# DiamondLightSource/fast-feedback-service

Hardware: AMD Instinct MI355X
Metric: detector frames/s (Eiger-16M 4362x4148 uint16) (higher is better)
Workload: dtype u16; 1 GPU; eiger16m: 4148x4362 uint16, 7x7 dispersion window, 32 frames/step/GPU resident in HBM, spots+centroids returned to host; streams=4, parallelism=single GPU, spot_gather=none (single GPU)

## Files before the change

### fast-feedback-service_amd/csrc/ffs_bench.hip

```cpp
#include "ffs_internal.hpp"

extern "C" int ffs_bench_threshold(ffs_stream* s, const void* device_pixels, size_t pitch, size_t fstride,
                                   uint32_t n_frames, uint32_t iters, float* ms_dense, float* ms_rest) {
    if (!s || !device_pixels || iters == 0) return FFS_ERR_INVALID;
    ffs_ctx* c = s->ctx;
    if (s->busy) {
        c->err = "stream busy";
        return FFS_ERR_INVALID;
    }
    int rc = check_layout(s, pitch, fstride, n_frames);
    if (rc != FFS_OK) return rc;
    HIP_TRY(c, hipSetDevice(c->device));
    s->batch_params = c->params;
    const bool ext = c->params.algorithm == FFS_ALGO_DISPERSION_EXTENDED;
    if (ext) {
        rc = ensure_extended_buffers(s);
        if (rc != FFS_OK) return rc;
    }
    s->ext_e_clean = false;
    const StreamGeometry geo = batch_stream_geometry(s, fstride, n_frames);
    ThresholdArgs ta = make_threshold_args(s, device_pixels, pitch, fstride, n_frames, geo, Rerun{});
    if (!ext && !win_default(c->params) && !window_kernel_for(s, ta)) {
        c->err = "ffs_bench_threshold: threshold_path 2 with a window other than 3,3 has no dense kernel to time";
        return FFS_ERR_INVALID;
    }
    const bool e_sparse = ext && ext_sparse_erode(c->tune);
    ta.eplane_clean = e_sparse ? 1 : 0;
    if (!ext) (void)wave_logs_for(s, ta, geo, Rerun{});
    const Layout& L = c->L;
    std::vector<hipEvent_t> ev(4 * (size_t)iters, nullptr);
    auto cleanup = [&]() { for (hipEvent_t e : ev) if (e) (void)hipEventDestroy(e); };
    for (auto& e : ev)
        if (hipEventCreate(&e) != hipSuccess) {
            cleanup();
            c->err = "hipEventCreate failed";
            return FFS_ERR_DEVICE;
        }
    (void)hipGetLastError();
    hipError_t err = hipSuccess;
    for (uint32_t i = 0; i < iters && err == hipSuccess; ++i) {
        err = hipMemsetAsync(s->d_bits, 0, (size_t)s->max_batch * L.plane_frame_stride, s->st);
        if (err == hipSuccess) err = hipMemsetAsync(s->d_tile_counts, 0, tile_counts_bytes(s), s->st);
        if (err == hipSuccess) err = hipMemsetAsync(s->d_occ, 0, (size_t)s->max_batch * occ_frame_words(L) * 4, s->st);
        if (err == hipSuccess && e_sparse) err = hipMemsetAsync(s->d_eplane, 0, (size_t)s->max_batch * L.plane_frame_stride, s->st);
        if (err != hipSuccess) break;
        launch_dense_kernel(s, ta, geo, n_frames, ev[4 * i], ev[4 * i + 1]);
        err = hipEventRecord(ev[4 * i + 2], s->st);
        launch_dense_rest(s, ta, n_frames);
        if (err == hipSuccess) err = hipEventRecord(ev[4 * i + 3], s->st);
        if (err == hipSuccess) err = hipGetLastError();
    }
    if (err == hipSuccess) err = hipMemsetAsync(s->d_overflow, 0, 4, s->st);
    if (err == hipSuccess) err = hipStreamSynchronize(s->st);
    double t_dense = 0, t_rest = 0;
    for (uint32_t i = 0; i < iters && err == hipSuccess; ++i) {
        float a = 0, b = 0;
        err = hipEventElapsedTime(&a, ev[4 * i], ev[4 * i + 1]);
        if (err == hipSuccess) err = hipEventElapsedTime(&b, ev[4 * i + 2], ev[4 * i + 3]);
        t_dense += a;
        t_rest += b;
    }
    cleanup();
    s->bits_dirty = true;
    s->counts_dirty = true;
    s->occ_dirty = true;
    if (err != hipSuccess) {
        c->err = std::string("ffs_bench_threshold: ") + hipGetErrorString(err);
        return FFS_ERR_DEVICE;
    }
    if (ms_dense) *ms_dense = (float)(t_dense / iters);
    if (ms_rest) *ms_rest = (float)(t_rest / iters);
    return FFS_OK;
}

static int bench_pipeline_impl(ffs_stream* const* streams, uint32_t n_streams, const void* device_pixels, size_t pitch, size_t fstride,
                               uint32_t n_frames, uint32_t steps, int64_t first_frame_id, uint64_t* n_boxes, uint64_t* n_strong) {
    uint64_t boxes = 0, strong = 0;
    std::vector<uint32_t> inflight;
    auto reap = [&]() -> int {
        const ffs_frame_result* res = nullptr;
        uint32_t n = 0;
        const int rc = ffs_wait_impl(streams[inflight.front()], &res, &n);
        inflight.erase(inflight.begin());
        if (rc != FFS_OK) return rc;
        for (uint32_t i = 0; i < n; ++i) { boxes += res[i].n_boxes; strong += res[i].num_strong_pixels; }
        return FFS_OK;
    };
    for (uint32_t step = 0; step < steps; ++step) {
        const uint32_t i = step % n_streams;
        if (inflight.size() == n_streams) {
            const int rc = reap();
            if (rc != FFS_OK) return rc;
        }
        const int rc = ffs_submit_device(streams[i], device_pixels, pitch, fstride, n_frames, first_frame_id + (int64_t)step * n_frames);
        if (rc != FFS_OK) return rc;
        inflight.push_back(i);
    }
    while (!inflight.empty()) {
        const int rc = reap();
        if (rc != FFS_OK) return rc;
    }
    if (n_boxes) *n_boxes = boxes;
    if (n_strong) *n_strong = strong;
    return FFS_OK;
// ... 86 lines not shown
```

### fast-feedback-service_amd/csrc/ffs_context.hip

```cpp
#include <sys/mman.h>

#include "ffs_internal.hpp"
#include "kernels_mask.hpp"

static_assert(sizeof(ReflOut) == sizeof(ffs_reflection), "record layout");
static_assert(offsetof(ReflOut, sum_intensity) == offsetof(ffs_reflection, sum_intensity), "record layout");

thread_local std::string g_create_error;

static void ctx_destroy_internal(ffs_ctx* c);
namespace {
struct Registry {
    std::mutex mu;
    std::unordered_set<const void*> live[3];
    std::atomic<bool> exiting{false};
    bool exit_hook_installed = false;
};
Registry& registry() {
    static Registry* r = new Registry();
    return *r;
}
static void on_process_exit() {
    Registry& r = registry();
    std::vector<ffs_ctx*> ctxs;
// ... 186 lines not shown
                {
                    std::unique_lock<std::mutex> lock(mu);
                    cv.wait(lock, [&] { return stop || generation != seen; });
                    if (stop) return;
                    seen = generation;
                    fn = job;
                    n = n_items;
                    if (fn) active.fetch_add(1);
                }
                if (!fn) continue;
                for (;;) {
                    const uint32_t i = next.fetch_add(1);
                    if (i >= n) break;
                    (*fn)(i);
                    done.fetch_add(1, std::memory_order_release);
                }
                active.fetch_sub(1, std::memory_order_release);
            }
        });
}
void AssemblyPool::run(uint32_t n, const std::function<void(uint32_t)>& fn) {
    {
        std::lock_guard<std::mutex> lock(mu);
        job = &fn;
        n_items = n;
        next.store(0);
        done.store(0);
        ++generation;
    }
    cv.notify_all();
    for (;;) {
        const uint32_t i = next.fetch_add(1);
        if (i >= n) break;
        fn(i);
        done.fetch_add(1, std::memory_order_release);
    }
    while (done.load(std::memory_order_acquire) < n) __builtin_ia32_pause();
    {
        std::lock_guard<std::mutex> lock(mu);
        job = nullptr;
    }
    while (active.load(std::memory_order_acquire) != 0) __builtin_ia32_pause();
}
void AssemblyPool::stop_and_join() {
    {
        std::lock_guard<std::mutex> lock(mu);
        stop = true;
    }
    cv.notify_all();
    for (auto& t : threads)
        if (t.joinable()) t.join();
}
AssemblyPool::~AssemblyPool() { stop_and_join(); }

extern "C" void ffs_ctx_destroy(ffs_ctx* c) {
    if (!c || !handle_take(kHandleCtx, c)) return;
    std::vector<ffs_stream*> streams;
    std::vector<ffs_stack3d*> stacks;
    {
        std::lock_guard<std::mutex> lock(c->stream_mu);
        streams.swap(c->live_streams);
        stacks.swap(c->live_stacks);
    }
    for (ffs_stream* s : streams)
        if (handle_take(kHandleStream, s)) stream_destroy_internal(s);
    for (ffs_stack3d* st : stacks)
        if (handle_take(kHandleStack, st)) {
            g_live_stacks.fetch_sub(1);
            stack3d_free(st);
        }
    ctx_destroy_internal(c);
}

static void ctx_destroy_internal(ffs_ctx* c) {
    (void)hipSetDevice(c->device);
    ahead_stop(c, true);
    for (auto* st : c->stack_pool) stack3d_free(st);
    c->stack_pool.clear();
    if (AssemblyPool* pool = c->assembly.exchange(nullptr)) {
        pool->owner.lock();
        pool->owner.unlock();
        delete pool;
    }
    if (c->d_maskbits) (void)hipFree(c->d_maskbits);
    if (c->d_ginfo) (void)hipFree(c->d_ginfo);
    if (c->d_mmap) (void)hipFree(c->d_mmap);
    if (c->dense_st) (void)hipStreamDestroy(c->dense_st);
    if (c->dense_st2) (void)hipStreamDestroy(c->dense_st2);
    if (c->d_handoff) (void)hipFree(c->d_handoff);
    if (c->up_st) (void)hipStreamDestroy(c->up_st);
    for (auto st : c->sparse_st) if (st) (void)hipStreamDestroy(st);
    for (auto e : c->chain_ev) if (e) (void)hipEventDestroy(e);
    for (auto& pb : c->pinned_pool) pinned_free(pb);
    delete c;
}

static int rebuild_mask_tables(ffs_ctx* c) {
    const Layout& L = c->L;
    const uint32_t gpitch = ginfo_pitch(L, c->pixel_bytes);
    HIP_TRY(c, hipMemset(c->d_ginfo, 0, (size_t)(L.H + kInfoExtraRows) * gpitch));
    const int groups = L.pitch_px / (c->pixel_bytes == 2 ? 8 : 4);
    (void)hipGetLastError();
    if (c->pixel_bytes == 2)
        hipLaunchKernelGGL(k_build_maps, dim3((groups + 255) / 256, L.H), dim3(256), 0, 0, c->d_maskbits, L.mpitch, L.W, L.H,
                           L.pitch_px, c->d_mmap, c->d_ginfo, gpitch);
    else
        hipLaunchKernelGGL(k_build_maps4, dim3((groups + 255) / 256, L.H), dim3(256), 0, 0, c->d_maskbits, L.mpitch, L.W, L.H,
                           L.pitch_px, c->d_mmap, c->d_ginfo, gpitch);
    HIP_TRY(c, hipGetLastError());
    HIP_TRY(c, hipDeviceSynchronize());
    return FFS_OK;
}

static int ffs_ctx_set_mask_impl(ffs_ctx* c, const uint8_t* host_mask) {
    if (!c) return FFS_ERR_INVALID;
    const Layout& L = c->L;
    std::vector<uint8_t> bits(L.plane_frame_stride, 0);
    const int full = L.W / 8;
    for (int y = 0; y < L.H; ++y) {
        uint8_t* row = bits.data() + (size_t)y * L.mpitch;
        if (host_mask) {
            const uint8_t* m = host_mask + (size_t)y * L.W;
            for (int g = 0; g < full; ++g) {
                uint64_t v;
                std::memcpy(&v, m + 8 * g, 8);
                const uint64_t nz = (((v & 0x7F7F7F7F7F7F7F7Full) + 0x7F7F7F7F7F7F7F7Full) | v) & 0x8080808080808080ull;
                row[g] = (uint8_t)(((nz >> 7) * 0x0102040810204080ull) >> 56);
            }
            for (int x = full * 8; x < L.W; ++x)
                if (m[x]) row[x >> 3] |= (uint8_t)(1u << (x & 7));
        } else {
            std::memset(row, 0xFF, (size_t)full);
            for (int x = full * 8; x < L.W; ++x) row[x >> 3] |= (uint8_t)(1u << (x & 7));
        }
    }
    HIP_TRY(c, hipSetDevice(c->device));
    HIP_TRY(c, hipMemcpy(c->d_maskbits, bits.data(), bits.size(), hipMemcpyHostToDevice));
    return rebuild_mask_tables(c);
}

static int ffs_ctx_get_mask_impl(ffs_ctx* c, uint8_t* host_mask) {
    if (!c || !host_mask) return FFS_ERR_INVALID;
    const Layout& L = c->L;
    std::vector<uint8_t> bits(L.plane_frame_stride);
    HIP_TRY(c, hipSetDevice(c->device));
    HIP_TRY(c, hipMemcpy(bits.data(), c->d_maskbits, bits.size(), hipMemcpyDeviceToHost));
    for (int y = 0; y < L.H; ++y)
        for (int x = 0; x < L.W; ++x)
            host_mask[(size_t)y * L.W + x] = (bits[(size_t)y * L.mpitch + (x >> 3)] >> (x & 7)) & 1;
    return FFS_OK;
}

extern "C" int ffs_ctx_apply_resolution_mask(ffs_ctx* c, float wavelength, float distance_m,
                                             float bcx, float bcy, float psx, float psy, float dmin,
                                             float dmax) {
    if (!c) return FFS_ERR_INVALID;
    HIP_TRY(c, hipSetDevice(c->device));
    const Layout& L = c->L;
    dim3 block(64, 1), grid((L.mpitch + 63) / 64, L.H);
    hipLaunchKernelGGL(k_resolution_mask, grid, block, 0, 0, c->d_maskbits, L.mpitch, L.W, L.H,
                       wavelength, distance_m, bcx, bcy, psx, psy, dmin, dmax);
    HIP_TRY(c, hipGetLastError());
    HIP_TRY(c, hipDeviceSynchronize());
    return rebuild_mask_tables(c);
}

extern "C" int ffs_ctx_set_params(ffs_ctx* c, const ffs_params* p) {
    if (!c || !p) return FFS_ERR_INVALID;
    if (p->kernel_half_x < 0 || p->kernel_half_x > kWinMaxHalf || p->kernel_half_y < 0 || p->kernel_half_y > kWinMaxHalf) {
        c->err = "ffs_ctx_set_params: kernel_half_x / kernel_half_y must be in 1..7 (0 = 3)";
        return FFS_ERR_INVALID;
    }
    const int win_px = (2 * win_half(p->kernel_half_x) + 1) * (2 * win_half(p->kernel_half_y) + 1);
    if (p->min_count < 2 || p->min_count > win_px || p->nsig_b < 0 || p->nsig_s < 0 || p->threshold < 0) {
        c->err = "ffs_ctx_set_params: need 2 <= min_count <= (2*kernel_half_x+1)*(2*kernel_half_y+1) (49 for the 7x7 window), "
                 "nsig_b >= 0, nsig_s >= 0, threshold >= 0";
        return FFS_ERR_INVALID;
    }
    if (p->algorithm == FFS_ALGO_DISPERSION_EXTENDED && !win_default(*p)) {
        c->err = "ffs_ctx_set_params: the extended dispersion algorithm needs the 7x7 window (kernel_half_x = kernel_half_y = 3): "
                 "its erosion and final pass derive from it";
        return FFS_ERR_INVALID;
    }
    if ((p->algorithm != FFS_ALGO_DISPERSION && p->algorithm != FFS_ALGO_DISPERSION_EXTENDED)
        || (p->extended_flavour != 0 && p->extended_flavour != 1)) {
        c->err = "ffs_ctx_set_params: unknown algorithm / extended_flavour";
        return FFS_ERR_INVALID;
    }
    c->params = *p;
    return FFS_OK;
}

extern "C" int ffs_ctx_device_layout(const ffs_ctx* c, size_t* pitch, size_t* fstride) {
    if (!c) return FFS_ERR_INVALID;
    if (pitch) *pitch = c->L.pitch;
    if (fstride) *fstride = c->L.frame_stride;
    return FFS_OK;
}

extern "C" int ffs_ctx_set_tuning(ffs_ctx* c, const char* key, long long value) {
    if (!c || !key) return FFS_ERR_INVALID;
    Tuning& t = c->tune;
    const std::string k = key;
    auto in = [&](long long lo, long long hi) { return value >= lo && value <= hi; };
    bool ok = true;
    if (k == "threshold_path") { if ((ok = in(0, 2))) t.threshold_path = (int)value; }
    else if (k == "window_kernel") { if ((ok = in(0, 1))) t.window_kernel = (int)value; }
    else if (k == "ext_first_pass") { if ((ok = value == 0 || value == 2)) t.ext_first_pass = (int)value; }
    else if (k == "sparse_stage") { if ((ok = in(1, 3))) t.sparse_stage = (int)value; }
    else if (k == "device_lists") { if ((ok = in(0, 2))) t.device_lists = (int)value; }
    else if (k == "strong_log") { if ((ok = in(0, 1))) t.strong_log = (int)value; }
    else if (k == "chain_runs") { if ((ok = in(0, 2))) t.chain_runs = (int)value; }
    else if (k == "dense_overlap") { if ((ok = in(0, 1))) t.dense_overlap = (int)value; }
    else if (k == "stream_prio") { if ((ok = in(0, 3))) t.stream_prio = (int)value; }
    else if (k == "wait_ahead") { if ((ok = in(0, 1))) t.wait_ahead = (int)value; }
    else if (k == "assembly_threads") { if ((ok = in(1, 31))) t.assembly_threads = (int)value; }
    else if (k == "sparse_bands") { if ((ok = in(0, 2))) t.sparse_bands = (int)value; }
    else if (k == "sparse_priority") {
        if ((ok = in(0, 2) && c->n_streams_made == 0)) {
            int lo = 0, hi = 0;
            HIP_TRY(c, hipSetDevice(c->device));
            HIP_TRY(c, hipDeviceGetStreamPriorityRange(&lo, &hi));
            const int prio = value == 0 ? hi : value == 1 ? lo : (lo + hi) / 2;
            for (auto& sp : c->sparse_st) {
                if (sp) (void)hipStreamDestroy(sp);
                sp = nullptr;
                HIP_TRY(c, hipStreamCreateWithPriority(&sp, hipStreamNonBlocking, prio));
            }
            t.sparse_priority = (int)value;
        }
    }
    else if (k == "sched") { if ((ok = (value == 0 || value == 3) && c->n_streams_made == 0)) t.sched = (int)value; }
    else if (k == "chain_first") { if ((ok = in(0, 64))) t.chain_first = (int)value; }
    else if (k == "bright_cap") { if ((ok = in(0, kBrightCap))) t.bright_cap = (int)value; }
    else if (k == "frames_per_group") { if ((ok = in(1, 1 << 30))) t.frames_per_group = (int)value; }
    else if (k == "target_waves") { if ((ok = in(1, 1 << 24))) t.target_waves = value; }
    else if (k == "stream_bands") { if ((ok = in(0, 4096))) t.stream_bands = (int)value; }
    else if (k == "dense_mask") { if ((ok = in(0, 1))) t.dense_mask = (int)value; }
    else if (k == "occupancy_bitmap") { if ((ok = in(0, 1))) t.occupancy_bitmap = (int)value; }
    else if (k == "direct_records") { if ((ok = in(0, 1) && c->n_streams_made == 0)) t.direct_records = (int)value; }
    else if (k == "decode_in_dense_stream") { if ((ok = in(0, 1))) t.decode_in_dense_stream = (int)value; }
    else if (k == "ext_fused") { if ((ok = in(0, 1))) t.ext_fused = (int)value; }
    else if (k == "ext_erode") { if ((ok = in(0, 2))) t.ext_erode = (int)value; }
    else if (k == "ext_e_sparse") { if ((ok = in(0, 1))) t.ext_e_sparse = (int)value; }
    else if (k == "ext_rest_aside") { if ((ok = in(0, 1))) t.ext_rest_aside = (int)value; }
    else if (k == "band_taper") { if ((ok = in(0, 99))) t.band_taper = (int)value; }
    else if (k == "rows_ahead") { if ((ok = in(2, 4))) t.rows_ahead = (int)value; }
    else if (k == "ccl_grid") { if ((ok = in(1, 1024))) t.ccl_grid = (int)value; }
    else {
        c->err = "ffs_ctx_set_tuning: unknown key '" + k + "'";
        return FFS_ERR_INVALID;
    }
    if (!ok) {
        c->err = "ffs_ctx_set_tuning: value out of range for '" + k + "' (sched / direct_records: before the first stream is created)";
        return FFS_ERR_INVALID;
    }
    return FFS_OK;
}


extern "C" void ffs_stream_destroy(ffs_stream* s) {
    if (!s || !handle_take(kHandleStream, s)) return;
    {
        ffs_ctx* c = s->ctx;
        std::lock_guard<std::mutex> lock(c->stream_mu);
        auto& v = c->live_streams;
        v.erase(std::remove(v.begin(), v.end(), s), v.end());
    }
    stream_destroy_internal(s);
}

void stream_destroy_internal(ffs_stream* s) {
    (void)hipSetDevice(s->ctx->device);
    if (s->job.joinable()) s->job.join();
    (void)ahead_take(s);
    gather_scratch_free(s);
    mark_idle(s);
#ifdef FFS_EXPERIMENTS
    if (s->phase_n) {
        const double k = 1.0 / (double)s->phase_n;
        std::fprintf(stderr, "[ffs exp] sparse launch, %llu frames: init %.1f | L1 / E %.1f | S + L2 %.1f | X U %.1f | P %.1f | R %.1f | whole %.1f us per frame\n",
                     s->phase_n, s->phase_sum[0] * k, s->phase_sum[1] * k, s->phase_sum[2] * k, s->phase_sum[3] * k, s->phase_sum[4] * k, s->phase_sum[5] * k, s->phase_sum[6] * k);
    }
    if (s->h_phase_ts) (void)hipHostFree(s->h_phase_ts);
#endif
    if (s->big) stream_destroy_internal(s->big);
    if (s->st_up && s->st_up != s->st) (void)hipStreamSynchronize(s->st_up);
    if (s->st) (void)hipStreamSynchronize(s->st);
    if (s->st_shared && s->ctx->dense_st2) (void)hipStreamSynchronize(s->ctx->dense_st2);
    if (s->st2 && s->st2 != s->st) { (void)hipStreamSynchronize(s->st2); if (!s->st2_shared) (void)hipStreamDestroy(s->st2); }
    if (s->h_pack_tab) (void)hipHostFree(s->h_pack_tab);
    void* dev[] = {s->d_slab, s->d_pack_k, s->d_pack_i, s->d_pack_tab, s->d_comp, s->d_tab, s->d_ext_pair[0], s->d_ext_pair[1], s->d_wlog, s->d_wlog_n, s->d_wpix,
                   s->d_band_hdr, s->d_band_acc, s->d_band_seam, s->d_bo_frames, s->d_bo_lane, s->d_bo_map, s->d_bo_state};
    for (void* p : dev)
        if (p) (void)hipFree(p);
    void* host[] = {s->h_tab, s->h_bo_frames, s->h_counts, s->h_recs, s->h_list_k, s->h_list_i, s->h_mask};
    for (void* p : host)
        if (p) (void)hipHostFree(p);
    if (s->h_img) {
        std::lock_guard<std::mutex> lock(s->ctx->stream_mu);
        s->ctx->pinned_pool.push_back(s->h_img_buf);
    }
    for (auto& e : s->ev)
        if (e) (void)hipEventDestroy(e);
    if (s->ev_pack) (void)hipEventDestroy(s->ev_pack);
    if (s->ev_sent) (void)hipEventDestroy(s->ev_sent);
    if (s->st && !s->st_shared) (void)hipStreamDestroy(s->st);
    delete s;
}

extern "C" int ffs_stream_create(ffs_ctx* c, ffs_stream** out) {
    if (!c || !out) return FFS_ERR_INVALID;
    const int rc = stream_create_sized(c, c->max_batch, c->cap, c->max_comp, out);
    if (rc != FFS_OK) return rc;
    {
        std::lock_guard<std::mutex> lock(c->stream_mu);
        c->live_streams.push_back(*out);
    }
    handle_add(kHandleStream, *out);
    return FFS_OK;
}

int stream_create_sized(ffs_ctx* c, uint32_t max_batch, uint32_t cap, uint32_t max_comp, ffs_stream** out) {
    *out = nullptr;
    HIP_TRY(c, hipSetDevice(c->device));
    ffs_stream* s = new (std::nothrow) ffs_stream();
    if (!s) return FFS_ERR_NOMEM;
    s->ctx = c;
    s->max_batch = max_batch;
// ... 192 lines not shown
```

### fast-feedback-service_amd/csrc/ffs_device.h

```cpp
#pragma once
#include <hip/hip_runtime.h>
#include <stdint.h>

#include "launch_geometry.hpp"

#ifdef FFS_EXPERIMENTS
#define FFS_DBG(args, bit) (((args).dbg & (bit)) != 0)
#define FFS_STOP_AFTER(A, phase) if ((A).stop_after == (phase)) return
#define FFS_PHASE_TS(A, idx) do { if ((A).phase_ts && threadIdx.x == 0) (A).phase_ts[(size_t)blockIdx.x * 8 + (idx)] = wall_clock64(); } while (0)
#else
#define FFS_PHASE_TS(A, idx) do {} while (0)
#define FFS_DBG(args, bit) false
#define FFS_STOP_AFTER(A, phase) do {} while (0)
#endif

namespace ffsamd {

constexpr int kInfoExtraRows = 3;

constexpr int kWlogCap = 256;
constexpr int kTileRows = 8;
constexpr int kExactListCap = 2048;

struct ThresholdArgs {
    const void* image;
    uint64_t frame_stride;
    uint32_t pitch;
    const uint8_t* maskbits;
    uint8_t* bits;
    uint8_t* strong_bytes;
    uint32_t* tile_counts;
    int W, H, pitch_px;
    uint32_t mpitch, bpitch;
    uint64_t plane_frame_stride, bytes_frame_stride;
    int n_strips, band_rows, n_bands, n_tiles;
    int band_rows2, band_split;
    float kS;
    float kB;
    int min_count;
    double nsig_b, nsig_s, threshold;
    double nsig_b2, nsig_s2;
    long long max_valid;
    int int_pred;
    uint32_t ib2, is2;
    uint32_t thr_floor;
    int bright_to_plane;
    uint8_t* dplane;
    uint8_t* eplane;
    int eplane_clean;
    int ext_strips, ext_band_rows, ext_bands;
    int ext_flavour;
    int ext_variant;
    const uint8_t* ginfo;
    const uint8_t* mmap;
    uint32_t gpitch;
    int gpf;
    int n_frames;
    int group_frames;
    int s_strips, s_band_rows, s_bands;
    uint32_t* bright_n;
    uint2* bright_list;
    uint32_t bright_cap;
    uint32_t* overflow;
    uint32_t* occ;
    uint32_t occ_frame_words;
    uint32_t occ_spr;
    int dense_mask;
    uint2* wlog;
    uint32_t* wlog_n;
    uint4* wpix;
    uint32_t* handoff;
    uint32_t handoff_seq;
    int dbg_prio;
    int dbg;
    int kx, ky;
    int w_strips, w_band_rows, w_bands;
    float w_kS, w_kB;
};

__host__ __device__ inline uint32_t stream_units(const ThresholdArgs& a) { return stream_units_of(a.n_bands, a.n_strips); }
__host__ __device__ inline uint32_t stream_chunk(const ThresholdArgs& a) { return stream_chunk_of(a.n_bands, a.n_strips); }
__device__ __forceinline__ bool stream_unit(const ThresholdArgs& a, uint32_t bid, int& strip, int& band) {
    return stream_unit_of(bid, a.n_bands, a.n_strips, strip, band);
}
__host__ __device__ inline uint32_t log_slot(const ThresholdArgs& a, uint32_t y, uint32_t band, uint32_t strip) {
    return log_slot_of(a.n_bands, a.n_strips, y, band, strip);
}

constexpr uint32_t kOvfStrongCap = 1u;
constexpr uint32_t kOvfCompCap = 2u;
constexpr uint32_t kOvfCorruptLz4 = 4u;
constexpr uint32_t kOvfBrightList = 8u;
constexpr uint32_t kOvfRuns = 16u;
constexpr uint32_t kOvfWaveLog = 32u;
constexpr uint32_t kOvfLdsForest = 64u;
constexpr uint32_t kOvfBandPlan = 128u;
constexpr uint32_t kOvfCorruptByteOffset = 256u;
constexpr uint32_t kRecTooSmall = 1u;
constexpr uint32_t kRecTooSpread = 2u;

constexpr int kSummaryWords = 8;
constexpr uint32_t kSumBoxes = 0, kSumStrongFiltered = 1, kSumReflections = 2, kSumFilteredSize = 3, kSumFilteredSep = 4;
__host__ __device__ constexpr size_t counts_strong_at(size_t) { return 0; }
__host__ __device__ constexpr size_t counts_comp_at(size_t B) { return B; }
__host__ __device__ constexpr size_t counts_summary_at(size_t B) { return 2 * B; }
__host__ __device__ constexpr size_t counts_status_at(size_t B) { return (2 + kSummaryWords) * B; }
__host__ __device__ constexpr size_t counts_frame_flags_at(size_t B) { return counts_status_at(B) + 1; }
__host__ __device__ constexpr size_t counts_device_words(size_t B) { return counts_status_at(B) + 1; }
__host__ __device__ constexpr size_t counts_host_words(size_t B) { return counts_frame_flags_at(B) + B; }

struct CompAcc2 {
    unsigned long long sum_i, sum_xi, sum_yi, peak;
    uint32_t x_min, x_max, y_min, y_max;
    uint32_t num_pixels, pad;
};

struct WireRec2 {
    uint16_t x_min, x_max, y_min, y_max;
    uint32_t npx_flags;
    float com_x, com_y;
    uint16_t peak_x, peak_y;
    uint32_t peak_intensity;
    float peak_centroid_distance;
    unsigned long long sum_intensity;
};

struct CclArgs {
    const void* image;
    uint64_t frame_stride;
    uint32_t pitch;
    uint8_t* bits;
    int clear_bits;
    const uint32_t* tile_counts;
    uint32_t* num_strong;
    uint32_t* row_off;
    uint32_t* list_k;
    uint32_t* list_i;
    uint32_t* parent;
    uint32_t* comp_id;
    uint32_t* n_comp;
    uint32_t* overflow;
    int W, H, pitch_px;
    uint32_t mpitch;
    uint64_t plane_frame_stride;
    int n_tiles;
    uint32_t cap;
    uint32_t max_comp;
    int pixel_bytes;
    CompAcc2* acc2;
    uint32_t* summary;
    uint8_t* strong_bytes;
    uint32_t bpitch;
    uint64_t bytes_frame_stride;
    int dense_bytes;
    int need_lists;
    uint32_t* occ;
    uint32_t occ_frame_words, occ_spr;
    int use_occ;
};

struct CompAcc {
    unsigned long long sum_i;
    unsigned long long sum_xi;
    unsigned long long sum_yi;
    unsigned long long sum_zi;
    unsigned long long peak;
// ... 58 lines not shown
```

### fast-feedback-service_amd/csrc/ffs_internal.hpp

```cpp
#pragma once
#include <algorithm>
#include <atomic>
#include <chrono>
#include <condition_variable>
#include <functional>
#include <cmath>
#include <cstdio>
#include <cstdlib>
#include <cstring>
#include <deque>
#include <map>
#include <mutex>
#include <new>
#include <string>
#include <thread>
#include <unordered_set>
#include <vector>

#include <hip/hip_runtime.h>
#include <hip/hip_ext.h>

#include "ffs_hip.h"
#include "ffs_device.h"
#include "tuning.hpp"
// ... 3 lines not shown
extern thread_local std::string g_create_error;

struct ThreadError {
    static std::string& text() {
        static thread_local std::string t;
        return t;
    }
    const ThreadError& operator=(const std::string& m) const { text() = m; return *this; }
    const ThreadError& operator=(const char* m) const { text() = m; return *this; }
    const char* c_str() const { return text().c_str(); }
    operator std::string() const { return text(); }
};


struct ffs_stack3d;

struct AssemblyPool {
    std::vector<std::thread> threads;
    std::mutex mu;
    std::condition_variable cv;
    std::mutex owner;
    const std::function<void(uint32_t)>* job = nullptr;
    uint32_t n_items = 0;
    std::atomic<uint32_t> next{0}, done{0};
    std::atomic<int> active{0};
    uint64_t generation = 0;
    bool stop = false;
    void start(int n_threads);
    void run(uint32_t n, const std::function<void(uint32_t)>& fn);
    void stop_and_join();
    ~AssemblyPool();
};

struct PinnedBuf {
    uint8_t* p = nullptr;
    size_t bytes = 0;
    void* map_base = nullptr;
    size_t map_len = 0;
};
PinnedBuf pinned_alloc(size_t bytes);
void pinned_free(PinnedBuf& b);

struct AheadThread {
    std::thread th;
    std::mutex mu;
    std::condition_variable cv_work, cv_done;
    std::deque<ffs_stream*> q;
    bool stop = false;
};

struct ffs_ctx {
    int device = 0;
    Tuning tune;
    Layout L{};
    int pixel_bytes = 2;
    uint32_t max_batch = 1;
    uint32_t cap = 0;
    uint32_t max_comp = 0;
    int n_tiles = 0;
    ffs_params params{};
    uint8_t* d_maskbits = nullptr;
    uint8_t* d_ginfo = nullptr;
    uint8_t* d_mmap = nullptr;
    hipStream_t dense_st = nullptr;
    hipStream_t dense_st2 = nullptr;
    uint32_t* d_handoff = nullptr;
    std::mutex dense_mu;
    uint32_t handoff_seq = 0;
    int handoff_last = -1;
    hipStream_t up_st = nullptr;
    hipStream_t sparse_st[2] = {nullptr, nullptr};
    int n_streams_made = 0;
    std::mutex stream_mu;
    std::vector<ffs_stream*> live_streams;
    std::vector<ffs_stack3d*> live_stacks;
    std::vector<ffs_stack3d*> stack_pool;
    std::vector<struct PinnedBuf> pinned_pool;
    std::atomic<int> inflight{0};
    static constexpr int kChainEvents = 16;
    hipEvent_t chain_ev[kChainEvents] = {};
    std::atomic<uint32_t> chain_ev_next{0};
    std::atomic<int> chain_ev_newest{-1};
    bool chain_ok = false;
    std::atomic<AssemblyPool*> assembly{nullptr};
    std::atomic<AheadThread*> ahead{nullptr};
    ThreadError err;
};

struct OverflowFrame;

constexpr uint32_t kBrightCap = 1u << 20;

struct ffs_stream {
    ffs_ctx* ctx = nullptr;
    uint32_t max_batch = 1;
    uint32_t cap = 0;
    uint32_t max_comp = 0;
    ffs_stream* big = nullptr;
    std::vector<OverflowFrame> ovf;
    bool lists_valid = true;
    bool log_off = false;
    uint2* d_wlog = nullptr;
    uint32_t* d_wlog_n = nullptr;
    uint4* d_wpix = nullptr;
    size_t wlog_waves = 0;
    uint4* d_band_hdr = nullptr;
    uint8_t* d_band_acc = nullptr;
    uint32_t* d_band_seam = nullptr;
    uint32_t band_slots = 0;
    uint32_t band_backoff = 0;
    uint32_t path_bits = 0;
    uint32_t reruns = 0;
    bool runs_overflowed = false;
    uint32_t *d_pack_k = nullptr, *d_pack_i = nullptr;
    StackSlice *d_pack_tab = nullptr, *h_pack_tab = nullptr;
    hipEvent_t ev_pack = nullptr;
    hipEvent_t ev_sent = nullptr;
    int ev_sent_dev = -1;
    bool sent_pending = false;
    hipStream_t st = nullptr;
    hipStream_t st_up = nullptr;
    bool st2_shared = false;
    bool st_shared = false;
    hipStream_t st2 = nullptr;
    hipEvent_t ev[7] = {};
    uint8_t* d_slab = nullptr;
    uint8_t* d_img = nullptr;
    uint8_t* d_bits = nullptr;
    uint8_t* d_sbytes = nullptr;
    uint8_t *d_dplane = nullptr, *d_eplane = nullptr;
    uint8_t* d_dplane2 = nullptr;
    uint8_t* d_eplane2 = nullptr;
    uint8_t* d_ext_pair[2] = {nullptr, nullptr};
    bool dplane2_clean = false;
    bool eplane2_clean = false;
    bool ext_e_clean = false;
    uint8_t* d_comp = nullptr;
    uint2 *d_tab = nullptr, *h_tab = nullptr;
    uint32_t dec_blocks = 0, dec_last = 0, dec_tail = 0, dec_block_elems = 0;
    uint4 *d_bo_frames = nullptr, *h_bo_frames = nullptr;
    uint2 *d_bo_lane = nullptr, *d_bo_map = nullptr;
    uint4* d_bo_state = nullptr;
    size_t bo_tiles_cap = 0;
    uint32_t spec_recs_per_frame = 256;
    uint64_t spec_recs_copied = 0;
    std::thread job;
    int job_rc = 0;
    std::string job_err;
    uint32_t *d_tile_counts = nullptr, *d_num_strong = nullptr, *d_row_off = nullptr;
    uint2* d_bright = nullptr;
    uint32_t *d_list_k = nullptr, *d_list_i = nullptr, *d_parent = nullptr;
    uint32_t *d_n_comp = nullptr, *d_overflow = nullptr, *d_summary = nullptr;
    CompAcc2* d_acc2 = nullptr;
    uint32_t* d_chunk_roots = nullptr;
    ReflOut* d_recs = nullptr;
    uint8_t* h_img = nullptr;
    size_t h_img_bytes = 0;
    PinnedBuf h_img_buf;
    size_t d_comp_bytes = 0;
    uint32_t* h_counts = nullptr;
    ReflOut* h_recs = nullptr;
    uint32_t* d_occ = nullptr;
    uint32_t* h_counts_dev = nullptr;
    bool ev1_pending = false;
    bool ev3_is_ev4 = false;
    bool dev_input = false;
// ... 31 lines not shown
    std::vector<float> centres_n;
    int ahead_state = 0;
};

struct OverflowFrame {
    uint32_t frame = 0;
    ffs_frame_result res{};
    std::vector<ffs_box> boxes;
    std::vector<ffs_reflection> refls;
    std::vector<uint32_t> k, inten;
};

static inline const OverflowFrame* overflow_frame(const std::vector<OverflowFrame>* ovf, uint32_t f) {
    if (ovf)
        for (const OverflowFrame& o : *ovf)
            if (o.frame == f) return &o;
    return nullptr;
}

template <typename F>
static int guarded(ffs_ctx* c, F&& body) {
    try {
        return body();
    } catch (const std::exception& e) {
        if (c) c->err = std::string("exception inside libffs_hip: ") + e.what();
        else g_create_error = std::string("exception inside libffs_hip: ") + e.what();
        return FFS_ERR_NOMEM;
    } catch (...) {
        if (c) c->err = "unknown exception inside libffs_hip";
        return FFS_ERR_NOMEM;
    }
}

#define HIP_TRY(ctx, expr)                                                              \
    do {                                                                                \
        hipError_t e_ = (expr);                                                         \
        if (e_ != hipSuccess) {                                                         \
            (ctx)->err = std::string(#expr) + ": " + hipGetErrorString(e_);             \
            return e_ == hipErrorOutOfMemory ? FFS_ERR_NOMEM : FFS_ERR_DEVICE;          \
        }                                                                               \
    } while (0)

struct Rerun {
    int threshold_path = -1;
    bool plane = false;
    bool no_bands = false;
    bool grid = false;
};
static inline bool ext_sparse_erode(const Tuning& t) { return t.ext_erode != 0 && t.ext_e_sparse; }
constexpr int kWinMaxHalf = 7;
static inline int win_half(int v) { return v ? v : 3; }
static inline bool win_default(const ffs_params& p) { return win_half(p.kernel_half_x) == 3 && win_half(p.kernel_half_y) == 3; }
static inline uint32_t occ_frame_words(const Layout& L) { return (uint32_t)(((uint64_t)L.H * (L.mpitch / 16) + 31) / 32 + 2); }
static inline size_t tile_counts_bytes(const ffs_stream* s) { return (((size_t)s->max_batch * s->ctx->n_tiles + 2) * 4 + 255) / 256 * 256; }
static inline void mark_busy(ffs_stream* s) {
    if (!s->busy) ++s->ctx->inflight;
    s->busy = true;
}
static inline void mark_idle(ffs_stream* s) {
    if (s->busy) --s->ctx->inflight;
    s->busy = false;
}
template <typename T>
static hipError_t dmalloc(T** p, size_t n_bytes) {
    return hipMalloc(reinterpret_cast<void**>(p), n_bytes + 256);
}

enum HandleKind { kHandleCtx = 0, kHandleStream = 1, kHandleStack = 2 };
void handle_add(HandleKind kind, const void* h);
bool handle_take(HandleKind kind, const void* h);
bool handle_live(HandleKind kind, const void* h);
bool process_exiting();
static inline bool stream_handle_ok(const ffs_stream* s) {
    if (handle_live(kHandleStream, s)) return true;
    g_create_error = "stale ffs_stream handle: the stream was destroyed (with its context, or by ffs_stream_destroy)";
    return false;
}
void stream_destroy_internal(ffs_stream* s);

int stream_create_sized(ffs_ctx* c, uint32_t max_batch, uint32_t cap, uint32_t max_comp, ffs_stream** out);
int ensure_host_staging(ffs_stream* s, size_t bytes);
size_t default_staging_bytes(const ffs_stream* s);
bool chain_prepare_device();
StreamGeometry batch_stream_geometry(const ffs_stream* s, size_t fstride, uint32_t n_frames);
ThresholdArgs make_threshold_args(ffs_stream* s, const void* img, size_t pitch, size_t fstride, uint32_t n_frames, const StreamGeometry& g, const Rerun& how);
int check_layout(ffs_stream* s, size_t pitch, size_t fstride, uint32_t n_frames);
int ensure_extended_buffers(ffs_stream* s);
int enqueue_batch(ffs_stream* s, const void* d_img, size_t pitch, size_t fstride, uint32_t n, const ffs_params* snapshot = nullptr,
                  const Rerun& how = Rerun{});
extern std::atomic<int> g_live_stacks;
bool wave_logs_for(ffs_stream* s, ThresholdArgs& a, const StreamGeometry& g, const Rerun& how);
void launch_dense_kernel(ffs_stream* s, const ThresholdArgs& a, const StreamGeometry& g, uint32_t n_frames, hipEvent_t start, hipEvent_t stop,
                         bool plane_clean = false, bool counts_clean = false);
void launch_dense_rest(ffs_stream* s, const ThresholdArgs& a, uint32_t n_frames);
bool window_kernel_for(const ffs_stream* s, const ThresholdArgs& a);
int ffs_wait_impl(ffs_stream* s, const ffs_frame_result** results, uint32_t* n_results);
void ahead_register(ffs_stream* s);
int ahead_take(ffs_stream* s);
void ahead_stop(ffs_ctx* c, bool destroy);
void stack3d_free(ffs_stack3d* st);
void gather_scratch_free(ffs_stream* s);
```

### fast-feedback-service_amd/csrc/ffs_submit.hip

```cpp
#include "ffs_internal.hpp"
#include "kernels_threshold.hpp"
#include "kernels_extended.hpp"
#include "kernels_stream.hpp"
#include "kernels_ccl.hpp"
#include "kernels_chain.hpp"
#include "kernels_band.hpp"
#include "kernels_decode.hpp"
#include "kernels_byteoffset.hpp"
#include "kernels_window.hpp"

bool chain_prepare_device() {
    const hipError_t e1 = hipFuncSetAttribute(reinterpret_cast<const void*>(&k_frame_chain<uint16_t>), hipFuncAttributeMaxDynamicSharedMemorySize, kChainDynBytes);
    const hipError_t e2 = hipFuncSetAttribute(reinterpret_cast<const void*>(&k_frame_chain<uint32_t>), hipFuncAttributeMaxDynamicSharedMemorySize, kChainDynBytes);
    const hipError_t e3 = hipFuncSetAttribute(reinterpret_cast<const void*>(&k_frame_chain<uint16_t, true>), hipFuncAttributeMaxDynamicSharedMemorySize, kChainDynBytes);
    const hipError_t e4 = hipFuncSetAttribute(reinterpret_cast<const void*>(&k_frame_chain<uint16_t, false, true>), hipFuncAttributeMaxDynamicSharedMemorySize, kChainDynBytes);
    const hipError_t e5 = hipFuncSetAttribute(reinterpret_cast<const void*>(&k_frame_chain<uint32_t, false, true>), hipFuncAttributeMaxDynamicSharedMemorySize, kChainDynBytes);
    (void)hipGetLastError();
    return e1 == hipSuccess && e2 == hipSuccess && e3 == hipSuccess && e4 == hipSuccess && e5 == hipSuccess;
}

static void set_buffers(ThresholdArgs& a, const ffs_stream* s, const void* img, size_t pitch, size_t fstride, const Rerun& how) {
    const ffs_ctx* c = s->ctx;
    const Layout& L = c->L;
    const ffs_params& p = s->batch_params;
    a.image = img;
    a.frame_stride = fstride;
    a.pitch = (uint32_t)pitch;
    a.maskbits = c->d_maskbits;
    a.bits = s->d_bits;
    a.strong_bytes = s->d_sbytes;
    a.tile_counts = s->d_tile_counts;
    a.W = L.W;
    a.H = L.H;
    a.pitch_px = L.pitch_px;
    a.mpitch = L.mpitch;
    a.bpitch = L.bpitch;
    a.plane_frame_stride = L.plane_frame_stride;
    a.bytes_frame_stride = L.bytes_frame_stride;
    a.n_tiles = c->n_tiles;
    a.bright_to_plane = how.threshold_path >= 0 ? how.threshold_path : c->tune.threshold_path;
    a.overflow = s->d_overflow;
    a.bright_n = s->d_tile_counts + tile_counts_bytes(s) / 4 - 1;
    a.bright_list = s->d_bright;
    a.bright_cap = std::min<uint32_t>(kBrightCap, (uint32_t)c->tune.bright_cap);
    a.occ = s->d_occ;
    a.occ_frame_words = occ_frame_words(L);
    a.occ_spr = L.mpitch / 16;
    a.dense_mask = (p.want_strong_mask || c->tune.dense_mask || a.bright_to_plane) ? 1 : 0;
#ifdef FFS_EXPERIMENTS
    a.dbg = c->tune.exp.k1_debug;
    if (a.dbg & 16) a.dense_mask = 1;
    if (a.dbg & 8) a.dense_mask = 0;
#endif
    a.dbg_prio = c->tune.stream_prio;
    a.ginfo = c->d_ginfo;
    a.mmap = c->d_mmap;
    a.gpitch = ginfo_pitch(L, c->pixel_bytes);
    a.gpf = groups_per_row(L, c->pixel_bytes);
    a.dplane = s->d_dplane;
    a.eplane = s->d_eplane;
    a.eplane_clean = s->ext_e_clean ? 1 : 0;
    a.ext_variant = (c->pixel_bytes == 2 && how.threshold_path < 0) ? c->tune.ext_first_pass : 0;
}
static void set_predicate(ThresholdArgs& a, const ffs_params& p) {
    a.kS = (float)(p.nsig_s * p.nsig_s * (1.0 - 1.0 / 65536.0));
    a.kB = (float)(p.nsig_b * (1.0 - 1.0 / 1048576.0));
    a.min_count = p.min_count;
    a.nsig_b = p.nsig_b;
    a.nsig_s = p.nsig_s;
    a.nsig_b2 = p.nsig_b * p.nsig_b;
    a.nsig_s2 = p.nsig_s * p.nsig_s;
    a.threshold = p.threshold;
    a.max_valid = p.max_valid;
    {
        const double b2 = p.nsig_b * p.nsig_b, s2 = p.nsig_s * p.nsig_s;
        a.int_pred = (b2 == std::floor(b2) && s2 == std::floor(s2) && b2 <= 1024.0 && s2 <= 1024.0 && p.threshold < 2147483648.0
                      && std::sqrt(b2) == p.nsig_b && std::sqrt(s2) == p.nsig_s) ? 1 : 0;
        a.ib2 = a.int_pred ? (uint32_t)b2 : 0u;
        a.is2 = a.int_pred ? (uint32_t)s2 : 0u;
        a.thr_floor = a.int_pred ? (uint32_t)std::floor(p.threshold) : 0u;
    }
    a.kx = win_half(p.kernel_half_x);
    a.ky = win_half(p.kernel_half_y);
    a.w_kS = (std::isfinite(p.nsig_s) && p.nsig_s <= 1024.0) ? (float)(p.nsig_s * p.nsig_s * (1.0 - 1.0 / 65536.0)) : 0.0f;
    a.w_kB = (std::isfinite(p.nsig_b) && p.nsig_b <= 1024.0) ? (float)(p.nsig_b * p.nsig_b * (1.0 - 1.0 / 65536.0)) : 0.0f;
    a.ext_flavour = p.extended_flavour;
}
static void set_geometry(ThresholdArgs& a, uint32_t n_frames, const StreamGeometry& g, const WindowGeometry& w, const ExtGeometry& e) {
    a.n_frames = (int)n_frames;
    a.group_frames = g.group_frames;
    a.n_strips = g.n_strips;
    a.n_bands = g.n_bands;
    a.band_rows = g.band_rows;
    a.band_rows2 = g.band_rows2;
    a.band_split = g.band_split;
    a.w_strips = w.w_strips;
    a.w_band_rows = w.w_band_rows;
    a.w_bands = w.w_bands;
    a.ext_strips = e.ext_strips;
    a.ext_band_rows = e.ext_band_rows;
    a.ext_bands = e.ext_bands;
}
StreamGeometry batch_stream_geometry(const ffs_stream* s, size_t fstride, uint32_t n_frames) {
    return stream_geometry(s->ctx->L, s->ctx->pixel_bytes, fstride, n_frames, s->ctx->tune);
}
ThresholdArgs make_threshold_args(ffs_stream* s, const void* img, size_t pitch, size_t fstride, uint32_t n_frames, const StreamGeometry& g, const Rerun& how) {
    ThresholdArgs a{};
    set_buffers(a, s, img, pitch, fstride, how);
    set_predicate(a, s->batch_params);
    set_geometry(a, n_frames, g, window_geometry(s->ctx->L, n_frames, a.ky), ext_geometry(s->ctx->L, n_frames));
    return a;
}

static dim3 stream_grid(const ThresholdArgs& a, const StreamGeometry& g) {
    return dim3(8u * stream_chunk(a), (unsigned)g.n_groups);
}

using StreamKernel = void (*)(ThresholdArgs);
static StreamKernel stream_kernel(const ffs_ctx* c, bool dense_mask, bool extended) {
    const int rows = std::clamp(c->tune.rows_ahead, 2, c->pixel_bytes == 4 ? 3 : 4);
    if (c->pixel_bytes == 4) return dense_mask ? k_stream_u32<2, true> : rows == 3 ? k_stream_u32<3, false> : k_stream_u32<2, false>;
    if (extended) return dense_mask ? k_stream_u16<2, true, true> : k_stream_u16<2, true, false>;
    if (dense_mask) return k_stream_u16<2, false, true>;
    return rows == 4 ? k_stream_u16<4, false, false> : rows == 3 ? k_stream_u16<3, false, false> : k_stream_u16<2, false, false>;
}
static void launch_stream(ffs_stream* s, const ThresholdArgs& a, const StreamGeometry& g, hipEvent_t start, hipEvent_t stop, hipStream_t st = nullptr) {
    hipExtLaunchKernelGGL(stream_kernel(s->ctx, a.dense_mask != 0, false), stream_grid(a, g), dim3(64), 0, st ? st : s->st, start, stop, 0, a);
}
bool window_kernel_for(const ffs_stream* s, const ThresholdArgs& a) {
    return s->batch_params.algorithm == FFS_ALGO_DISPERSION && a.bright_to_plane != 2
           && (!win_default(s->batch_params) || s->ctx->tune.window_kernel == 1);
}
template <typename PixelT>
static void launch_window_t(const ThresholdArgs& a, dim3 grid, hipStream_t st, hipEvent_t start, hipEvent_t stop) {
    const size_t lds = win_ring_bytes((int)sizeof(PixelT), a.ky);
    switch (a.kx) {
        case 1: hipExtLaunchKernelGGL((k_window<PixelT, 1>), grid, dim3(64), lds, st, start, stop, 0, a); break;
        case 2: hipExtLaunchKernelGGL((k_window<PixelT, 2>), grid, dim3(64), lds, st, start, stop, 0, a); break;
        case 3: hipExtLaunchKernelGGL((k_window<PixelT, 3>), grid, dim3(64), lds, st, start, stop, 0, a); break;
        case 4: hipExtLaunchKernelGGL((k_window<PixelT, 4>), grid, dim3(64), lds, st, start, stop, 0, a); break;
        case 5: hipExtLaunchKernelGGL((k_window<PixelT, 5>), grid, dim3(64), lds, st, start, stop, 0, a); break;
        case 6: hipExtLaunchKernelGGL((k_window<PixelT, 6>), grid, dim3(64), lds, st, start, stop, 0, a); break;
        default: hipExtLaunchKernelGGL((k_window<PixelT, 7>), grid, dim3(64), lds, st, start, stop, 0, a); break;
    }
}
static void launch_window(ffs_stream* s, const ThresholdArgs& a, uint32_t n_frames, hipEvent_t start, hipEvent_t stop, hipStream_t st = nullptr) {
    const dim3 grid((unsigned)(a.w_strips * a.w_bands), n_frames);
    if (!st) st = s->st;
    if (s->ctx->pixel_bytes == 4) launch_window_t<uint32_t>(a, grid, st, start, stop);
    else launch_window_t<uint16_t>(a, grid, st, start, stop);
}
static void launch_bright_fix(ffs_stream* s, const ThresholdArgs& a, hipStream_t st) {
    if (s->ctx->pixel_bytes == 4) hipLaunchKernelGGL(k_bright_fix<uint32_t>, dim3(32), dim3(256), 0, st, a);
    else hipLaunchKernelGGL(k_bright_fix<uint16_t>, dim3(32), dim3(256), 0, st, a);
}
static void launch_exact(ffs_stream* s, const ThresholdArgs& a, uint32_t n_frames, hipStream_t st) {
    const dim3 grid((unsigned)a.n_tiles, n_frames);
    if (a.kx != 3 || a.ky != 3) {
        if (s->ctx->pixel_bytes == 4) hipLaunchKernelGGL(k_exact_w<uint32_t>, grid, dim3(256), 0, st, a);
        else hipLaunchKernelGGL(k_exact_w<uint16_t>, grid, dim3(256), 0, st, a);
        return;
    }
    if (s->ctx->pixel_bytes == 4) hipLaunchKernelGGL(k_exact<uint32_t>, grid, dim3(256), 0, st, a);
    else hipLaunchKernelGGL(k_exact<uint16_t>, grid, dim3(256), 0, st, a);
}

static bool ext_stream_first(const ThresholdArgs& a) { return a.ext_variant >= 2; }

static void launch_ext_first(ffs_stream* s, const ThresholdArgs& a, const StreamGeometry& g, uint32_t n_frames, hipEvent_t start, hipEvent_t stop, bool fix_here = true,
                             bool plane_clean = false, bool counts_clean = false) {
    if (ext_stream_first(a)) {
        if (!plane_clean) (void)hipMemsetAsync(a.dplane, 0, (size_t)n_frames * a.plane_frame_stride, s->st);
        if (!counts_clean) (void)hipMemsetAsync(a.tile_counts, 0, tile_counts_bytes(s), s->st);
        hipExtLaunchKernelGGL(stream_kernel(s->ctx, a.dense_mask != 0, true), stream_grid(a, g), dim3(64), 0, s->st, start, stop, 0, a);
        if (fix_here) hipLaunchKernelGGL((k_bright_fix<uint16_t, true>), dim3(32), dim3(256), 0, s->st, a);
        return;
    }
    dim3 g1((unsigned)(a.ext_strips * a.ext_bands), n_frames);
    if (s->ctx->pixel_bytes == 2) hipExtLaunchKernelGGL(k_ext_first<uint16_t>, g1, dim3(64), 0, s->st, start, stop, 0, a);
    else hipExtLaunchKernelGGL(k_ext_first<uint32_t>, g1, dim3(64), 0, s->st, start, stop, 0, a);
}
static void launch_ext_rest(ffs_stream* s, const ThresholdArgs& a, uint32_t n_frames, hipStream_t st) {
    const bool u16 = s->ctx->pixel_bytes == 2;
    if (!ext_stream_first(a)) (void)hipMemsetAsync(a.strong_bytes, 0, (size_t)n_frames * a.bytes_frame_stride, st);
    dim3 g3((unsigned)a.n_tiles, n_frames);
    if (u16 && s->ctx->tune.ext_fused) {
        hipLaunchKernelGGL(k_ext_erode_final, g3, dim3(256), (size_t)(kTileRows + 10) * a.mpitch, st, a);
        return;
    }
    const int erode = s->ctx->tune.ext_erode;
    if (erode != 0) {
        const unsigned strips = (a.mpitch / 4 + 61) / 62, rows = erode == 1 ? 32 : 16;
        const dim3 ge(strips * 8u * (((unsigned)((a.H + rows - 1) / rows) + 7u) / 8u), n_frames);
// ... 54 lines not shown
    return true;
}
bool wave_logs_for(ffs_stream* s, ThresholdArgs& a, const StreamGeometry& g, const Rerun& how) {
    if (!wave_logs_possible(s, a, how)) return false;
    size_t slots = stream_log_slots(g);
    if (slots > s->wlog_waves) slots = std::max(slots, max_stream_log_slots(s->ctx->L, s->ctx->pixel_bytes, a.frame_stride, s->max_batch, s->ctx->tune));
    if (!ensure_wave_logs(s, slots)) return false;
    a.wlog = s->d_wlog;
    a.wlog_n = s->d_wlog_n;
    a.wpix = s->d_wpix;
    return true;
}

void launch_dense_kernel(ffs_stream* s, const ThresholdArgs& a, const StreamGeometry& g, uint32_t n_frames, hipEvent_t start, hipEvent_t stop, bool plane_clean, bool counts_clean) {
    if (s->batch_params.algorithm == FFS_ALGO_DISPERSION_EXTENDED) launch_ext_first(s, a, g, n_frames, start, stop, true, plane_clean, counts_clean);
    else if (window_kernel_for(s, a)) launch_window(s, a, n_frames, start, stop);
    else launch_stream(s, a, g, start, stop);
}
void launch_dense_rest(ffs_stream* s, const ThresholdArgs& a, uint32_t n_frames) {
    if (s->batch_params.algorithm == FFS_ALGO_DISPERSION_EXTENDED) launch_ext_rest(s, a, n_frames, s->st);
    else if (window_kernel_for(s, a)) return;
    else if (a.bright_to_plane) launch_exact(s, a, n_frames, s->st);
    else if (!a.wlog) launch_bright_fix(s, a, s->st);
}

int check_layout(ffs_stream* s, size_t pitch, size_t fstride, uint32_t n_frames) {
    ffs_ctx* c = s->ctx;
    if (n_frames == 0 || n_frames > s->max_batch) {
        c->err = "n_frames must be in 1..max_batch";
        return FFS_ERR_INVALID;
    }
    if (pitch % 16 || pitch < (size_t)c->L.pitch_px * c->pixel_bytes || pitch >= (1ull << 32)
        || fstride < pitch * c->L.H || (pitch * c->L.H) >= (1ull << 32)) {
        c->err = "device layout: pitch must be a multiple of 16 bytes and >= round_up(width,128)*pixel_bytes; "
                 "frame_stride >= pitch*height";
        return FFS_ERR_INVALID;
    }
    return FFS_OK;
}

#ifdef FFS_EXPERIMENTS
__global__ void k_dummy_spin(uint32_t ticks, uint32_t* sink) {
    extern __shared__ uint32_t s_dummy[];
    const uint64_t t0 = wall_clock64();
    uint32_t it = 0;
    while (wall_clock64() - t0 < ticks && it < (1u << 20)) { __builtin_amdgcn_s_sleep(20); ++it; }
    if (it == 0xFFFFFFFFu) { s_dummy[threadIdx.x] = it; *sink = s_dummy[0]; }
}
#endif

static bool ensure_band_buffers(ffs_stream* s, uint32_t slots) {
    if (slots <= s->band_slots) return true;
    if (s->d_band_hdr) {
        (void)hipFree(s->d_band_hdr); (void)hipFree(s->d_band_acc); (void)hipFree(s->d_band_seam);
        s->d_band_hdr = nullptr; s->d_band_acc = nullptr; s->d_band_seam = nullptr;
    }
    s->band_slots = 0;
    if (hipMalloc(reinterpret_cast<void**>(&s->d_band_hdr), (size_t)slots * sizeof(uint4)) != hipSuccess
        || hipMalloc(reinterpret_cast<void**>(&s->d_band_acc), (size_t)slots * kBandCompStride * sizeof(ChainAcc)) != hipSuccess
        || hipMalloc(reinterpret_cast<void**>(&s->d_band_seam), (size_t)slots * 2 * kBandSeamCap * 4) != hipSuccess) {
        (void)hipGetLastError();
        return false;
    }
    s->band_slots = slots;
    return true;
}
static bool band_stage_for(ffs_stream* s, const StreamGeometry& g, size_t fstride, uint32_t n_frames) {
    const ffs_ctx* c = s->ctx;
    if (!band_plan_holds(g, c->L, c->pixel_bytes)) return false;
    uint32_t slots = band_slots(g, n_frames);
    if (slots > s->band_slots) slots = std::max(slots, max_band_slots(c->L, c->pixel_bytes, fstride, s->max_batch, c->tune));
    return ensure_band_buffers(s, slots);
}


#define FFS_TRY(expr)                    \
    do {                                 \
        const int rc_ = (expr);          \
        if (rc_ != FFS_OK) return rc_;   \
    } while (0)

struct BatchPlan {
    uint32_t n = 0;
    bool wait_upload = false;
    bool counts_were_clean = false;
    bool ext = false;
    bool ext_sparse_erode = false;
    bool window = false;
    bool list_path = false;
    bool aside = false;
    bool will_chain = false;
    bool runs_ok = false;
    bool dense_batch = false;
    bool use_log = false;
    bool runs_launch = false;
    bool need_lists = false;
    bool banded = false;
    bool chain_first = false;
    bool want_dense_bytes = false;
    StreamGeometry geo{};
    ThresholdArgs ta{};
    ThresholdArgs ta_launch{};
    BandSplit band;
    uint32_t path_bits = 0;
};

static BatchPlan plan_batch(ffs_stream* s, const void* d_img, size_t pitch, size_t fstride, uint32_t n, const Rerun& how) {
    ffs_ctx* c = s->ctx;
    const Layout& L = c->L;
    const ffs_params& p = s->batch_params;
    BatchPlan P;
    P.n = n;
    P.wait_upload = s->st_up != s->st && !s->dev_input;
    P.counts_were_clean = !s->counts_dirty;
    P.ext = p.algorithm == FFS_ALGO_DISPERSION_EXTENDED;
    P.ext_sparse_erode = ext_sparse_erode(c->tune);
    P.geo = batch_stream_geometry(s, fstride, n);
    P.ta = make_threshold_args(s, d_img, pitch, fstride, n, P.geo, how);
    P.window = !P.ext && window_kernel_for(s, P.ta);
    P.list_path = !P.ext && !P.ta.bright_to_plane && !P.window;
    P.want_dense_bytes = P.window ? (p.want_strong_mask || c->tune.dense_mask)
                                  : (P.list_path || (P.ext && ext_stream_first(P.ta))) ? P.ta.dense_mask != 0 : true;
    const bool can_chain = c->tune.sparse_stage >= 2 && L.H <= 65535 && c->chain_ok && s->direct_recs && s->h_counts_dev
                           && c->n_tiles <= kChainMaxTiles && L.H <= kChainMaxRows;
    P.runs_ok = c->pixel_bytes == 2 && L.W <= kChainRunMaxW && c->tune.chain_runs != 0 && !s->runs_overflowed;
    if (can_chain && c->tune.sparse_stage == 2 && s->n_frames > 0) {
        uint32_t prev_max = 0;
        for (uint32_t f = 0; f < s->n_frames; ++f) prev_max = std::max(prev_max, s->h_counts[counts_strong_at(s->max_batch) + f]);
        P.dense_batch = prev_max > (uint32_t)kChainLdsEntries;
    }
    P.will_chain = can_chain && (!P.dense_batch || P.runs_ok) && !how.grid;
    P.ta_launch = P.ta;
    P.use_log = P.list_path && P.will_chain && !P.dense_batch && wave_logs_for(s, P.ta_launch, P.geo, how);
#ifdef FFS_EXPERIMENTS
    if (c->tune.exp.chain_skip) P.will_chain = false;
#endif
    P.runs_launch = P.will_chain && !P.use_log && P.runs_ok && (P.dense_batch || c->tune.chain_runs == 2);
    P.aside = !P.ext && s->st2 != s->st;
    const int depth = c->inflight.load() + (s->busy ? 0 : 1);
    P.need_lists = p.want_strong_list || c->tune.device_lists == 1 || (c->tune.device_lists == 2 && g_live_stacks.load() > 0);
    const bool depth_ok = c->tune.sparse_bands >= 2 || depth >= 4 || depth <= 1 || c->n_streams_made >= 4;
    P.banded = P.use_log && c->tune.sparse_bands != 0 && depth_ok && !P.need_lists && !P.ta.dense_mask && !how.no_bands && s->band_backoff == 0
               && band_stage_for(s, P.geo, fstride, n);
    if (P.banded) P.band = band_split(P.geo);
    P.chain_first = P.list_path && P.aside && P.will_chain && !P.banded && c->tune.chain_first > 0 && depth <= c->tune.chain_first;
    P.path_bits = (P.use_log ? FFS_PATH_WAVE_LOGS : 0u) | (P.will_chain && !P.banded ? FFS_PATH_FRAME_CHAIN : 0u) | (P.banded ? FFS_PATH_BANDS : 0u)
                  | (P.runs_launch ? FFS_PATH_RUNS : 0u) | (!P.will_chain ? FFS_PATH_GRID_KERNELS : 0u) | (P.ext ? FFS_PATH_EXTENDED : 0u)
                  | (P.window ? FFS_PATH_WINDOW : 0u);
    return P;
}

static int take_extended_planes(ffs_stream* s, bool& plane_clean) {
    plane_clean = false;
    s->ext_e_clean = false;
    if (s->batch_params.algorithm != FFS_ALGO_DISPERSION_EXTENDED) return FFS_OK;
    FFS_TRY(ensure_extended_buffers(s));
    std::swap(s->d_dplane, s->d_dplane2);
    std::swap(s->d_eplane, s->d_eplane2);
    plane_clean = s->dplane2_clean;
    s->ext_e_clean = s->dplane2_clean && s->eplane2_clean && ext_sparse_erode(s->ctx->tune);
    s->dplane2_clean = false;
    s->eplane2_clean = false;
    return FFS_OK;
}

static int reset_for_batch(ffs_stream* s, const BatchPlan& plan, bool& dense_resets) {
    ffs_ctx* c = s->ctx;
    const Layout& L = c->L;
    dense_resets = false;
    if (plan.wait_upload && plan.ext) HIP_TRY(c, hipStreamWaitEvent(s->st, s->ev[1], 0));
    if (!plan.ext && s->bits_dirty) {
        HIP_TRY(c, hipMemsetAsync(s->d_bits, 0, (size_t)s->max_batch * L.plane_frame_stride, s->st));
        dense_resets = true;
    }
    if (!plan.ext && s->counts_dirty) {
        HIP_TRY(c, hipMemsetAsync(s->d_tile_counts, 0, tile_counts_bytes(s), s->st));
        dense_resets = true;
    }
    if (s->occ_dirty) {
        HIP_TRY(c, hipMemsetAsync(s->d_occ, 0, (size_t)s->max_batch * occ_frame_words(L) * 4, s->st));
        s->occ_dirty = false;
        dense_resets = true;
    }
    s->counts_dirty = true;
    s->bits_dirty = true;
    return FFS_OK;
}

static int wait_for_upload(ffs_stream* s, const BatchPlan& plan, hipStream_t st) {
    if (plan.wait_upload) HIP_TRY(s->ctx, hipStreamWaitEvent(st, s->ev[1], 0));
    return FFS_OK;
}
static int sparse_stream_follows(ffs_stream* s, bool ev2_on_dispatch) {
    if (!ev2_on_dispatch) HIP_TRY(s->ctx, hipEventRecord(s->ev[2], s->st));
    if (s->st2 != s->st) HIP_TRY(s->ctx, hipStreamWaitEvent(s->st2, s->ev[2], 0));
    return FFS_OK;
}

static int launch_stream_overlapped(ffs_stream* s, const BatchPlan& plan, hipEvent_t ev_start, bool& launched) {
    ffs_ctx* c = s->ctx;
    launched = false;
// ... 198 lines not shown
            BA.sub = plan.band.sub;
            BA.sub_rows = plan.band.sub_rows;
            const dim3 gb((unsigned)(plan.ta_launch.n_bands * BA.sub), n);
            if (c->pixel_bytes == 2) hipExtLaunchKernelGGL(k_band_cc<uint16_t>, gb, dim3(64), 0, s->st2, c->chain_ev[slot], nullptr, 0, BA);
            else hipExtLaunchKernelGGL(k_band_cc<uint32_t>, gb, dim3(64), 0, s->st2, c->chain_ev[slot], nullptr, 0, BA);
            hipLaunchKernelGGL(k_frame_merge, dim3(n), dim3(kMergeThreads), 0, s->st2, BA);
        } else {
            hipExtLaunchKernelGGL(frame_chain_kernel(plan, c->pixel_bytes), dim3(n), dim3(kChainThreads), kChainDynBytes, s->st2, c->chain_ev[slot], nullptr, 0, A);
        }
        if (plan.aside) c->chain_ev_newest.store(slot);
    }
    HIP_TRY(c, hipGetLastError());
    if (plan.ext && ext_stream_first(plan.ta) && s->st2 != s->st) {
        HIP_TRY(c, hipMemsetAsync(s->d_dplane2, 0, (size_t)s->max_batch * c->L.plane_frame_stride * (plan.ext_sparse_erode ? 2u : 1u), s->st2));
        s->dplane2_clean = true;
        s->eplane2_clean = plan.ext_sparse_erode;
    }
    HIP_TRY(c, hipEventRecord(s->ev[4], s->st2));
    s->ev3_is_ev4 = true;
    s->spec_recs_copied = (uint64_t)s->max_batch * s->max_comp;
    return finish_enqueue(s, n, plan.ext, false);
}

static int launch_grid_stage(ffs_stream* s, const BatchPlan& plan, const CclArgs& ca, SegArgs sa) {
    ffs_ctx* c = s->ctx;
    const uint32_t n = plan.n;
    bool skip_sparse = false;
#ifdef FFS_EXPERIMENTS
    if (c->tune.exp.chain_skip) {
        skip_sparse = true;
        if (c->tune.exp.dummy_us > 0)
            hipLaunchKernelGGL(k_dummy_spin, dim3(c->tune.exp.dummy_wg), dim3(c->tune.exp.dummy_threads),
                               (size_t)c->tune.exp.dummy_lds, s->st2, (uint32_t)c->tune.exp.dummy_us * 100u, s->d_tile_counts);
    }
#endif
    if (!skip_sparse) {
        sa.recs = s->direct_recs ? (void*)s->h_recs_dev : (void*)s->d_recs;
        sa.chunk_roots = s->d_chunk_roots;
        sa.chunks_max = s->cap / kRootChunk + 1;
        const dim3 gseg((unsigned)c->tune.ccl_grid, n), b256(256);
        if (c->pixel_bytes == 2) hipLaunchKernelGGL(k_emit_list_w<uint16_t>, dim3(c->n_tiles, n), dim3(64), 0, s->st2, ca);
        else hipLaunchKernelGGL(k_emit_list_w<uint32_t>, dim3(c->n_tiles, n), dim3(64), 0, s->st2, ca);
        hipLaunchKernelGGL(k_union<false>, gseg, b256, 0, s->st2, sa);
        hipLaunchKernelGGL(k_reduce_roots, gseg, b256, 0, s->st2, sa);
        hipLaunchKernelGGL(k_finalize_roots, gseg, b256, 0, s->st2, sa);
    }
    HIP_TRY(c, hipGetLastError());
    HIP_TRY(c, hipEventRecord(s->ev[3], s->st2));
    s->ev3_is_ev4 = false;

    const size_t B = s->max_batch;
    HIP_TRY(c, hipMemcpyAsync(s->h_counts, s->d_num_strong, counts_device_words(B) * 4, hipMemcpyDeviceToHost, s->st2));
    if (s->direct_recs) {
        s->spec_recs_copied = (uint64_t)B * s->max_comp;
    } else {
        s->spec_recs_copied = std::min<uint64_t>((uint64_t)s->spec_recs_per_frame * n, (uint64_t)B * s->max_comp);
        HIP_TRY(c, hipMemcpyAsync(s->h_recs, s->d_recs, s->spec_recs_copied * sizeof(WireRec2), hipMemcpyDeviceToHost, s->st2));
    }
    HIP_TRY(c, hipEventRecord(s->ev[4], s->st2));
    return finish_enqueue(s, n, plan.ext || skip_sparse, skip_sparse);
}

static int launch_sparse_stage(ffs_stream* s, const BatchPlan& plan) {
    const CclArgs ca = make_ccl_args(s, plan);
    const SegArgs sa = make_seg_args(s, plan);
    s->bits_cleared = ca.clear_bits != 0;
    s->lists_valid = !(plan.use_log || plan.runs_launch) || plan.need_lists;
    s->dense_valid = plan.want_dense_bytes;
    s->occ_dirty = !(ca.use_occ && plan.will_chain);
    s->chain_mode = plan.will_chain;
    s->path_bits = plan.path_bits;
    return plan.will_chain ? launch_one_launch_stage(s, plan, ca, sa) : launch_grid_stage(s, plan, ca, sa);
}

int enqueue_batch(ffs_stream* s, const void* d_img, size_t pitch, size_t fstride, uint32_t n, const ffs_params* snapshot, const Rerun& how) {
    s->batch_params = snapshot ? *snapshot : s->ctx->params;
    s->cur_img = d_img;
    s->cur_pitch = pitch;
    s->cur_fstride = fstride;
    (void)hipGetLastError();
    bool ext_plane_clean = false;
    FFS_TRY(take_extended_planes(s, ext_plane_clean));
    const BatchPlan plan = plan_batch(s, d_img, pitch, fstride, n, how);
    if (plan.use_log && s->band_backoff > 0 && !how.no_bands) --s->band_backoff;
    bool dense_resets = false;
    FFS_TRY(reset_for_batch(s, plan, dense_resets));
    FFS_TRY(launch_threshold_stage(s, plan, dense_resets, ext_plane_clean));
    return launch_sparse_stage(s, plan);
}

extern "C" int ffs_submit_device(ffs_stream* s, const void* device_pixels, size_t pitch, size_t fstride,
                                 uint32_t n_frames, int64_t first_frame_id) {
    if (!s || !device_pixels || !stream_handle_ok(s)) return FFS_ERR_INVALID;
    ffs_ctx* c = s->ctx;
    if (s->busy) {
        c->err = "stream already has a batch in flight: call ffs_wait() first";
        return FFS_ERR_INVALID;
    }
    int rc = check_layout(s, pitch, fstride, n_frames);
    if (rc != FFS_OK) return rc;
    HIP_TRY(c, hipSetDevice(c->device));
    s->dev_input = true;
    s->ev1_pending = true;
    s->first_id = first_frame_id;
    s->reruns = 0;
    rc = enqueue_batch(s, device_pixels, pitch, fstride, n_frames);
    if (rc == FFS_OK) ahead_register(s);
    return rc;
}

extern "C" int ffs_submit(ffs_stream* s, const void* host_pixels, uint32_t n_frames, int64_t first_frame_id) {
    if (!s || !host_pixels || !stream_handle_ok(s)) return FFS_ERR_INVALID;
    ffs_ctx* c = s->ctx;
    if (s->busy) {
        c->err = "stream already has a batch in flight: call ffs_wait() first";
        return FFS_ERR_INVALID;
    }
    if (n_frames == 0 || n_frames > s->max_batch) {
        c->err = "n_frames must be in 1..max_batch";
        return FFS_ERR_INVALID;
    }
    const Layout& L = c->L;
    HIP_TRY(c, hipSetDevice(c->device));
    s->dev_input = false;
    HIP_TRY(c, hipEventRecord(s->ev[0], s->st_up));
    const size_t row = (size_t)L.W * c->pixel_bytes;
    HIP_TRY(c, hipMemcpy2DAsync(s->d_img, L.pitch, host_pixels, row, row, (size_t)L.H * n_frames,
                                hipMemcpyHostToDevice, s->st_up));
    HIP_TRY(c, hipEventRecord(s->ev[1], s->st_up));
    s->first_id = first_frame_id;
    s->reruns = 0;
    const int rc = enqueue_batch(s, s->d_img, L.pitch, L.frame_stride, n_frames);
    if (rc == FFS_OK) ahead_register(s);
    return rc;
}



static int ensure_decode_buffers(ffs_stream* s) {
    ffs_ctx* c = s->ctx;
    if (s->d_tab) return FFS_OK;
    const size_t es = c->pixel_bytes, nelem = (size_t)c->L.W * c->L.H;
    const size_t block = (size_t)kDecBlockBytes / es;
    const size_t n_full = nelem / block, rem = nelem - n_full * block;
    s->dec_block_elems = (uint32_t)block;
    s->dec_blocks = (uint32_t)(n_full + (rem >= 8 ? 1 : 0));
    s->dec_last = (uint32_t)(rem >= 8 ? rem / 8 * 8 : block);
    s->dec_tail = (uint32_t)(rem % 8);
    const size_t tab_bytes = (size_t)s->max_batch * (s->dec_blocks + 1) * sizeof(uint2);
    if (dmalloc(&s->d_tab, tab_bytes) != hipSuccess
        || hipHostMalloc(reinterpret_cast<void**>(&s->h_tab), tab_bytes, hipHostMallocDefault) != hipSuccess) {
        (void)hipGetLastError();
        c->err = "allocation of the compressed-chunk buffers failed";
        return FFS_ERR_NOMEM;
    }
    return FFS_OK;
}

static inline uint32_t be32(const uint8_t* p) {
    return ((uint32_t)p[0] << 24) | ((uint32_t)p[1] << 16) | ((uint32_t)p[2] << 8) | p[3];
}

static int stage_chunks(ffs_stream* s, int codec, const void* const* chunks, const size_t* chunk_bytes, uint32_t n,
                        std::vector<size_t>& base) {
    ffs_ctx* c = s->ctx;
    const Layout& L = c->L;
// ... 370 lines not shown
```

### fast-feedback-service_amd/csrc/kernels_band.hpp

```cpp
#pragma once
#include "kernels_chain.hpp"

namespace ffsamd {

constexpr int kBandChunks = 8;
constexpr int kBandEntries = 64 * kBandChunks;
constexpr int kBandPx = 768;
constexpr int kBandPer = kBandPx / 64;
constexpr int kBandSlots = 64;
constexpr int kBandCompStride = 256;
constexpr int kBandSeamCap = 256;
constexpr int kBandItems = (kBandPx - kBandEntries) / 2;
constexpr int kMergeThreads = 256;
constexpr int kMergeCap = 4096;
constexpr int kMergeSeamLds = 8;
constexpr int kMergeLabels = 2;
constexpr int kMergePer = kMergeCap / kMergeThreads;
static_assert(sizeof(ChainAcc) == 56 && kBandSlots * (int)sizeof(ChainAcc) <= kBandCw * 4, "the accumulators take the counters' LDS");
static_assert(kBandEntries + 2 * kBandItems <= kBandPx && kBandMaxRows % 2 == 0, "LDS plan");

struct BandArgs {
    ChainArgs A;
    int sub, sub_rows;
    uint4* hdr;
    ChainAcc* acc;
    uint32_t* seam;
};

template <typename PixelT>
__global__ __launch_bounds__(64) void k_band_cc(const BandArgs B) {
    const ThresholdArgs& T = B.A.t;
    const CclArgs& a = B.A.c;
    if (T.dbg_prio & 2) __builtin_amdgcn_s_setprio(3);
    __shared__ uint32_t s_lst[16];
    __shared__ uint32_t s_row[kBandMaxRows + 2];
    __shared__ __align__(16) uint32_t s_cw[kBandCw];
    __shared__ __align__(8) uint2 s_ent[kBandEntries];
    __shared__ uint16_t s_x[kBandPx];
    __shared__ uint8_t s_y[kBandPx];
    __shared__ PixelT s_i[kBandPx];
    __shared__ uint32_t s_par[kBandPx];
    __shared__ uint32_t s_flag;

    const int band = (int)blockIdx.x / B.sub, sub = (int)blockIdx.x - band * B.sub, frame = blockIdx.y, lane = threadIdx.x;
    const uint32_t W = (uint32_t)a.W;
    constexpr uint32_t kGroupPx = sizeof(PixelT) == 2 ? 8u : 4u;
    const uint32_t l_y = (uint32_t)frame / (uint32_t)T.group_frames;
    const uint32_t l_fe = (uint32_t)frame - l_y * (uint32_t)T.group_frames;
    const uint32_t gsep = (uint32_t)T.gpf + 1u, G0 = l_fe * gsep, G1 = G0 + (uint32_t)T.gpf - 1u;
    const uint32_t l_s0 = G0 / (uint32_t)kSOwned;
    const uint32_t l_ns = min(G1 / (uint32_t)kSOwned - l_s0 + 1u, 16u);
    const uint32_t wave0 = log_slot(T, l_y, (uint32_t)band, l_s0);
    const int sb1 = min(band_first_row(band + 1, T.band_rows, T.band_rows2, T.band_split), a.H);
    const int yb0 = min(band_first_row(band, T.band_rows, T.band_rows2, T.band_split) + sub * B.sub_rows, sb1);
    const int yb1 = min(yb0 + B.sub_rows, sb1);
    const uint32_t rows = (uint32_t)(yb1 - yb0);
    const uint8_t* img = (const uint8_t*)a.image + (uint64_t)frame * a.frame_stride;
    const size_t slot = (size_t)frame * (size_t)gridDim.x + (size_t)blockIdx.x;

    FFS_STOP_AFTER(B.A, 10);
    if (lane == 0) s_flag = (rows > (uint32_t)kBandMaxRows || rows * l_ns > (uint32_t)kBandCw) ? kOvfBandPlan : 0u;
    for (uint32_t i = lane; i < min(rows * l_ns, (uint32_t)kBandCw); i += 64) s_cw[i] = 0;
    for (uint32_t i = lane; i < kBandEntries; i += 64) s_par[i] = 0;
    __syncthreads();

    uint32_t cnt = 0;
    if ((uint32_t)lane < l_ns && rows != 0) {
        cnt = T.wlog_n[wave0 + (uint32_t)lane];
        if (cnt > (uint32_t)kWlogCap) { atomicOr(&s_flag, kOvfWaveLog); cnt = (uint32_t)kWlogCap; }
    }
    const uint32_t incl0 = wave_inclusive_scan(cnt);
    if (lane < 16) s_lst[lane] = incl0 - cnt;
    const uint32_t nb = (uint32_t)__builtin_amdgcn_readlane((int)incl0, 63);
    if (nb > (uint32_t)kBandEntries) atomicOr(&s_flag, kOvfBandPlan);
    __syncthreads();
    uint32_t n = 0, ncomp = 0, n_top = 0, n_bot = 0;
    if (s_flag == 0 && nb != 0) {
        {
            uint2 ent[kBandChunks];
#pragma unroll
            for (int c = 0; c < kBandChunks; ++c) {
                const uint32_t f = (uint32_t)(c * 64 + lane);
                ent[c] = make_uint2(0xFFFFFFFFu, 0xFFFF0000u);
                if (f < nb) {
                    uint32_t k = 0;
                    for (uint32_t j = 1; j < l_ns; ++j) k += f >= s_lst[j] ? 1u : 0u;
                    ent[c] = T.wlog[(uint64_t)(wave0 + k) * kWlogCap + (f - s_lst[k])];
                    ent[c].y = ((ent[c].y >> 16) != l_fe || (int)(ent[c].x >> 16) < yb0 || (int)(ent[c].x >> 16) >= yb1) ? 0xFFFF0000u : (k << 16) | (ent[c].y & 0xFFFFu);
                }
            }
#pragma unroll
            for (int c = 0; c < kBandChunks; ++c)
                if ((uint32_t)(c * 64) < nb) s_ent[c * 64 + lane] = ent[c];
        }
        __syncthreads();
        FFS_STOP_AFTER(B.A, 12);
        const uint32_t nchunks = (nb + 63u) / 64u;
        auto mine_of = [](uint2 v) -> bool { return (v.y >> 16) != 0xFFFFu; };
        auto load_px = [&](uint32_t c) -> uint4 {
            uint4 px = make_uint4(0u, 0u, 0u, 0u);
            if (c < nchunks) {
                const uint32_t f = c * 64u + (uint32_t)lane;
                const uint2 v = s_ent[f];
                if (f < nb && mine_of(v) && (v.y & 0xFFFFu)) px = T.wpix[(uint64_t)(wave0 + (v.y >> 16)) * kWlogCap + (f - s_lst[v.y >> 16])];
            }
            return px;
        };
        const uint4 px0 = load_px(0), px1 = load_px(1);

        {
            uint32_t* items = s_par + kBandEntries;
            uint32_t nm = 0;
            for (uint32_t c = 0; c < nchunks; ++c) {
                const uint2 v = s_ent[c * 64 + lane];
                uint32_t maybe = mine_of(v) ? (v.y >> 8) & 0xFFu & ~v.y : 0u;
                const uint32_t pc = (uint32_t)__popc(maybe);
                const uint32_t inc = wave_inclusive_scan(pc);
                uint32_t q = nm + inc - pc;
                nm += (uint32_t)__builtin_amdgcn_readlane((int)inc, 63);
                while (maybe) {
                    const int b = __ffs((int)maybe) - 1;
                    maybe &= maybe - 1;
                    if (q < (uint32_t)kBandItems) {
                        items[2 * q] = v.x;
                        items[2 * q + 1] = ((c * 64u + (uint32_t)lane) << 3) | (uint32_t)b;
                    }
                    ++q;
                }
            }
            if (nm > (uint32_t)kBandItems) atomicOr(&s_flag, kOvfBandPlan);
            if (nm != 0) {
                __syncthreads();
                for (uint32_t i = lane; i < min(nm, (uint32_t)kBandItems); i += 64) {
                    const uint32_t rg = items[2 * i], sb = items[2 * i + 1];
                    const uint32_t row = rg >> 16, ge = rg & 0xFFFFu, b = sb & 7u;
                    if (exact_strong_lite<PixelT>(T, img, (int)(ge * kGroupPx + b), (int)row)) atomicOr(&s_par[sb >> 3], 1u << b);
                }
// ... 184 lines not shown
                        uint32_t* dst = reinterpret_cast<uint32_t*>(out + c0);
                        const uint32_t* src = reinterpret_cast<const uint32_t*>(s_acc);
                        for (uint32_t w = lane; w < ndw; w += 64) dst[w] = src[w];
                    }
                    __syncthreads();
                }
                n_top = s_row[1] - s_row[0];
                n_bot = s_row[rows] - s_row[rows - 1];
                if (n_top > (uint32_t)kBandSeamCap || n_bot > (uint32_t)kBandSeamCap) atomicOr(&s_flag, kOvfBandPlan);
                uint32_t* seam = B.seam + slot * 2 * kBandSeamCap;
                for (uint32_t j = lane; j < min(n_top, (uint32_t)kBandSeamCap); j += 64) seam[j] = (uint32_t)s_x[j] | ((uint32_t)s_id[j] << 16);
                const uint32_t bb = s_row[rows - 1];
                for (uint32_t j = lane; j < min(n_bot, (uint32_t)kBandSeamCap); j += 64) seam[kBandSeamCap + j] = (uint32_t)s_x[bb + j] | ((uint32_t)s_id[bb + j] << 16);
            }
        }
    }
    __syncthreads();
    if (lane == 0) B.hdr[slot] = make_uint4(n, ncomp, n_top | (n_bot << 16), s_flag | (rows << 16));
}
template __global__ void k_band_cc<uint16_t>(const BandArgs);
template __global__ void k_band_cc<uint32_t>(const BandArgs);

__global__ __launch_bounds__(kMergeThreads) void k_frame_merge(const BandArgs B) {
    const ChainArgs& A = B.A;
    const CclArgs& a = A.c;
    const SegArgs& sa = A.s;
    const ThresholdArgs& T = A.t;
    if (T.dbg_prio & 2) __builtin_amdgcn_s_setprio(3);
    __shared__ uint32_t s_off[kMergeMaxBands + 1];
    __shared__ uint32_t s_par[kMergeCap];
    __shared__ uint16_t s_l2id[kMergeCap];
    __shared__ uint32_t s_touched[kMergeCap / 32];
    __shared__ uint32_t s_wave[kMergeThreads / 64];
    __shared__ uint32_t s_sm[kSummaryWords];
    __shared__ uint32_t s_tot[2];
    __shared__ __align__(16) uint32_t s_out[kMergeLabels * kMergeThreads * (sizeof(WireRec2) / 4)];
    __shared__ __align__(16) uint32_t s_seam[kMergeMaxBands * 2 * kMergeSeamLds];
    const int frame = blockIdx.x, tid = threadIdx.x;
    const uint32_t W = (uint32_t)a.W;
    const uint32_t nbands = (uint32_t)(T.n_bands * B.sub);
    const uint4* hdr = B.hdr + (size_t)frame * nbands;
    ChainAcc* acc = B.acc + (size_t)frame * nbands * kBandCompStride;
    const uint32_t* seam = B.seam + (size_t)frame * nbands * 2 * kBandSeamCap;

    FFS_PHASE_TS(A, 0);
    FFS_STOP_AFTER(A, 10);
    FFS_STOP_AFTER(A, 11);
    FFS_STOP_AFTER(A, 12);
    FFS_STOP_AFTER(A, 13);
    if (tid < kSummaryWords) s_sm[tid] = 0;
    if (tid < 2) s_tot[tid] = 0;
    for (int i = tid; i < kMergeCap / 32; i += kMergeThreads) s_touched[i] = 0;
    __syncthreads();
    uint4 h = make_uint4(0u, 0u, 0u, 0u);
    if ((uint32_t)tid < nbands) h = hdr[tid];
    for (uint32_t j = (uint32_t)tid; j < nbands * 2u * (kMergeSeamLds / 4); j += kMergeThreads) {
        const uint32_t list = j / (kMergeSeamLds / 4), q = j % (kMergeSeamLds / 4);
        reinterpret_cast<uint4*>(s_seam)[j] = reinterpret_cast<const uint4*>(seam + (size_t)list * kBandSeamCap)[q];
    }
    if (h.x) atomicAdd(&s_tot[0], h.x);
    if (h.w & 0xFFFFu) atomicOr(&s_tot[1], h.w & 0xFFFFu);
    uint32_t NB;
    const uint32_t my_off = block_exclusive_scan<kMergeThreads>(h.y, s_wave, NB);
    if ((uint32_t)tid < nbands) s_off[tid] = my_off;
    if (tid == 0) s_off[nbands] = NB;
    __syncthreads();
    const uint32_t total = s_tot[0];
    uint32_t flags = s_tot[1];
    if (NB > (uint32_t)kMergeCap) flags |= kOvfBandPlan;
    FFS_PHASE_TS(A, 1);
    uint32_t before = 0;

    if (flags == 0) {
        const uint32_t per = (NB + kMergeThreads - 1) / kMergeThreads;
        const uint32_t i0 = min((uint32_t)tid * per, NB), i1 = min(i0 + per, NB);
        for (uint32_t i = i0; i < i1; ++i) s_par[i] = i;
        __syncthreads();
        if ((uint32_t)tid + 1 < nbands && (h.z >> 16) != 0u) {
            const uint32_t b = (uint32_t)tid;
            uint32_t t = b + 1;
            uint4 ht = hdr[t];
            while ((ht.w >> 16) == 0u && t + 1 < nbands) ht = hdr[++t];
            const uint32_t nbot = h.z >> 16, ntop = (ht.w >> 16) != 0u ? ht.z & 0xFFFFu : 0u;
            if (nbot && ntop) {
                const uint32_t* bot = seam + ((size_t)b * 2 + 1) * kBandSeamCap;
                const uint32_t* top = seam + ((size_t)t * 2) * kBandSeamCap;
                const uint32_t* lbot = s_seam + (b * 2u + 1u) * kMergeSeamLds;
                const uint32_t* ltop = s_seam + (t * 2u) * kMergeSeamLds;
                auto bot_at = [&](uint32_t i) -> uint32_t { return i < (uint32_t)kMergeSeamLds ? lbot[i] : bot[i]; };
                auto top_at = [&](uint32_t i) -> uint32_t { return i < (uint32_t)kMergeSeamLds ? ltop[i] : top[i]; };
                const uint32_t ob = s_off[b], ot = s_off[t];
                const uint32_t last = bot_at(nbot - 1), first = top_at(0);
                if ((last & 0xFFFFu) == W - 1 && (first & 0xFFFFu) == 0u) uf_union(s_par, ob + (last >> 16), ot + (first >> 16));
                uint32_t p = 0, q = 0;
                uint32_t vb = bot_at(0), vt = first;
                for (;;) {
                    const uint32_t xb = vb & 0xFFFFu, xt = vt & 0xFFFFu;
                    if (xb == xt) uf_union(s_par, ob + (vb >> 16), ot + (vt >> 16));
                    if (xb <= xt) { if (++p >= nbot) break; vb = bot_at(p); }
                    else { if (++q >= ntop) break; vt = top_at(q); }
                }
            }
        }
        __syncthreads();
        FFS_PHASE_TS(A, 2);
        auto acc_of = [&](uint32_t id) -> ChainAcc* {
            uint32_t lo = 0, hi = nbands - 1;
            while (lo < hi) {
                const uint32_t mid = lo + ((hi - lo + 1) >> 1);
                if (s_off[mid] <= id) lo = mid; else hi = mid - 1;
            }
            return acc + (size_t)lo * kBandCompStride + (id - s_off[lo]);
        };
        uint32_t mine = 0;
        for (uint32_t i = i0; i < i1; ++i) {
            const uint32_t root = uf_find(s_par, i);
            if (root == i) {
                ++mine;
            } else {
                atomicOr(&s_touched[root >> 5], 1u << (root & 31u));
                const ChainAcc m = *acc_of(i);
                ChainAcc* r = acc_of(root);
                atomicMin(&r->x_min, m.x_min); atomicMax(&r->x_max, m.x_max);
                atomicMin(&r->y_min, m.y_min); atomicMax(&r->y_max, m.y_max);
                atomicAdd(&r->num_pixels, m.num_pixels);
                atomicAdd(&r->sum_i, m.sum_i);
                atomicAdd(&r->sum_xi, m.sum_xi);
                atomicAdd(&r->sum_yi, m.sum_yi);
                atomicMax(&r->peak, m.peak);
            }
        }
        __syncthreads();
        FFS_PHASE_TS(A, 3);
        {
            uint32_t sl = block_exclusive_scan<kMergeThreads>(mine, s_wave, before);
            for (uint32_t i = i0; i < i1; ++i)
                if (s_par[i] == i) {
                    if (sl < (uint32_t)kMergeCap) s_l2id[sl] = (uint16_t)i;
                    ++sl;
                }
        }
        __syncthreads();
        FFS_PHASE_TS(A, 4);
        WireRec2* recs = reinterpret_cast<WireRec2*>(sa.recs) + (uint64_t)frame * A.rec_stride;
        const uint32_t ncomp = min(before, sa.max_comp);
        constexpr uint32_t kRound = (uint32_t)(kMergeLabels * kMergeThreads);
        for (uint32_t L0 = 0; L0 < ncomp; L0 += kRound) {
            unsigned long long v[kMergeLabels][7];
#pragma unroll
            for (int u = 0; u < kMergeLabels; ++u) {
                const uint32_t lab = L0 + (uint32_t)(u * kMergeThreads + tid);
                if (lab < ncomp) {
                    const uint32_t id = s_l2id[lab];
                    const unsigned long long* p = reinterpret_cast<const unsigned long long*>(acc_of(id));
                    if ((s_touched[id >> 5] >> (id & 31u)) & 1u) {
#pragma unroll
                        for (int w = 0; w < 7; ++w) v[u][w] = __hip_atomic_load(p + w, __ATOMIC_RELAXED, __HIP_MEMORY_SCOPE_AGENT);
                    } else {
#pragma unroll
                        for (int w = 0; w < 7; ++w) v[u][w] = p[w];
                    }
                }
            }
#pragma unroll
            for (int u = 0; u < kMergeLabels; ++u) {
                const uint32_t slot = (uint32_t)(u * kMergeThreads + tid);
                if (L0 + slot < ncomp) {
// ... 24 lines not shown
```

### fast-feedback-service_amd/csrc/kernels_chain.hpp

```cpp
#pragma once
#include "kernels_ccl.hpp"
#include "kernels_threshold.hpp"

namespace ffsamd {

constexpr int kChainThreads = 1024;
constexpr int kChainWaves = kChainThreads / 64;
constexpr int kChainMaxRows = 4480;
constexpr int kChainMaxTiles = kChainMaxRows / kTileRows;
constexpr int kChainListCap = 320;
constexpr int kChainSegCap = 512;
constexpr int kChainQuads = 4;
constexpr int kChainLdsEntries = 20480;
constexpr int kChainPer = kChainLdsEntries / kChainThreads;
constexpr int kChainSlots = 832;
constexpr int kChainRunCap = 16384;
constexpr int kChainRunPer = kChainRunCap / kChainThreads;
constexpr int kChainRunMaxW = 16383;

struct ChainAcc {
    unsigned long long sum_i, sum_xi, sum_yi, peak;
    uint32_t x_min, x_max, y_min, y_max;
    uint32_t num_pixels, pad;
};
// ... 455 lines not shown
#pragma unroll
                    for (int c = 0; c < 4; ++c)
                        buf[q][c] = __builtin_amdgcn_raw_buffer_load_b32(r_words, off, (uint32_t)c * 256u, 0);
                }
            };
            auto stage_batch = [&](int b, const uint32_t (&buf)[kChainQuads][4]) {
#pragma unroll
                for (int q = 0; q < kChainQuads; ++q) {
                    const int r = b * kChainQuads + q;
                    if (__builtin_amdgcn_ballot_w64((buf[q][0] | buf[q][1] | buf[q][2] | buf[q][3]) != 0u) == 0ull) continue;
                    if (n_list + 256 > kChainListCap) drain(false);
#pragma unroll
                    for (int c = 0; c < 4; ++c) {
                        const uint32_t w = buf[q][c];
                        const unsigned long long nz = __builtin_amdgcn_ballot_w64(w != 0u);
                        if (nz == 0ull) continue;
                        if (w) {
                            const int e = n_list + (int)__builtin_amdgcn_mbcnt_hi((uint32_t)(nz >> 32), __builtin_amdgcn_mbcnt_lo((uint32_t)nz, 0u));
                            s_g[e] = (uint32_t)(r * 256 + c * 64 + lane);
                            s_w[e] = w;
                        }
                        n_list += __popcll(nz);
                    }
                }
            };
            uint32_t b0[kChainQuads][4], b1[kChainQuads][4], b2[kChainQuads][4];
            const int nbatches = (nrounds + kChainQuads - 1) / kChainQuads;
            load_batch(0, b0);
            load_batch(1, b1);
            for (int b = 0; b < nbatches; b += 3) {
                load_batch(b + 2, b2);
                stage_batch(b, b0);
                load_batch(b + 3, b0);
                stage_batch(b + 1, b1);
                load_batch(b + 4, b1);
                stage_batch(b + 2, b2);
            }
            drain(true);
            }
            if (lane == 0) s_wrun[wave] = rrun - s_toff[tb];
        }
    }
    __syncthreads();
    FFS_STOP_AFTER(A, 2);
    FFS_PHASE_TS(A, 2);

    {
        constexpr int kPerRow = (kChainMaxRows + 1 + kChainThreads - 1) / kChainThreads;
        const int y0 = min(tid * kPerRow, a.H + 1), y1 = min(y0 + kPerRow, a.H + 1);
        uint32_t loc[kPerRow];
        uint32_t mine = 0;
#pragma unroll
        for (int q = 0; q < kPerRow; ++q) {
            loc[q] = y0 + q < y1 ? s_row[y0 + q] : 0u;
            mine += loc[q];
        }
        uint32_t tot;
        uint32_t run = block_exclusive_scan<kChainThreads>(mine, s_wave, tot);
#pragma unroll
        for (int q = 0; q < kPerRow; ++q) {
            if (y0 + q < y1) {
                s_row[y0 + q] = min(run, a.cap);
                run += loc[q];
            }
        }
        if constexpr (LOG) {
            total = tot;
            n = min(total, a.cap);
            in_lds = n <= (uint32_t)kChainLdsEntries;
        }
    }
    __syncthreads();
    if constexpr (LOG) {
        run_flag |= s_flag;
        if (!in_lds) run_flag |= kOvfLdsForest;
        if (run_flag == 0 && total != 0) {
            constexpr int kMaxStrips = 16;
            uint16_t* s_x = reinterpret_cast<uint16_t*>(s_dyn + kChainStageOff);
            uint32_t* cw = reinterpret_cast<uint32_t*>(s_big) + (size_t)wave * (kChainForestBytes / 4 / kChainWaves);
            const int cw_rows = (kChainForestBytes / 4 / kChainWaves) / kMaxStrips;
            uint8_t* sbytes = a.strong_bytes + (uint64_t)frame * a.bytes_frame_stride;
            const uint32_t ns = min(l_ns, (uint32_t)kMaxStrips);
            for (int band = wave; band < T.n_bands; band += kChainWaves) {
                const int yb0 = band_first_row(band, T.band_rows, T.band_rows2, T.band_split);
                const int yb1 = min(band_first_row(band + 1, T.band_rows, T.band_rows2, T.band_split), (int)a.H);
                for (int r0 = yb0; r0 < yb1; r0 += cw_rows) {
                    const int r1 = min(r0 + cw_rows, yb1);
                    for (int i = lane; i < (r1 - r0) * kMaxStrips; i += 64) cw[i] = 0;
                    __builtin_amdgcn_wave_barrier();
                    const uint32_t nb = band_begin(band);
                    const bool one = nb <= 64u * kLogChunks;
                    uint2 ent[kLogChunks];
                    for (uint32_t sb = 0; sb < nb; sb += 64 * kLogChunks) {
                        load_chunks(band, sb, nb, ent);
#pragma unroll
                        for (int c = 0; c < kLogChunks; ++c) {
                            const uint2 v = ent[c];
                            const int row = (int)(v.x >> 16);
                            if ((v.y >> 16) != l_fe || row < r0 || row >= r1) continue;
                            uint32_t k, e;
                            (void)band_entry(sb + (uint32_t)(c * 64 + lane), nb, k, e);
                            if (k < ns) atomicAdd(&cw[(row - r0) * kMaxStrips + (int)k], (uint32_t)__popc(v.y & 0xFFu));
                        }
                    }
                    __builtin_amdgcn_wave_barrier();
                    for (int r = r0 + lane; r < r1; r += 64) {
                        uint32_t at = s_row[r];
                        for (uint32_t k = 0; k < ns; ++k) {
                            const uint32_t c = cw[(r - r0) * kMaxStrips + (int)k];
                            cw[(r - r0) * kMaxStrips + (int)k] = at;
                            at += c;
                        }
                    }
                    __builtin_amdgcn_wave_barrier();
                    for (uint32_t sb = 0; sb < nb; sb += 64 * kLogChunks) {
                        if (!one) load_chunks(band, sb, nb, ent);
#pragma unroll
                        for (int c = 0; c < kLogChunks; ++c) {
                            if (sb + (uint32_t)(c * 64) >= nb) break;
                            const uint2 v = ent[c];
                            uint32_t k, e;
                            const bool have = band_entry(sb + (uint32_t)(c * 64 + lane), nb, k, e);
                            const int row = (int)(v.x >> 16);
                            const bool mine = have && (v.y >> 16) == l_fe && row >= r0 && row < r1 && k < ns;
                            uint4 px = make_uint4(0u, 0u, 0u, 0u);
                            if (mine) px = T.wpix[(uint64_t)log_wave(band, k) * kWlogCap + e];
                            const uint32_t cb = mine ? v.y & 0xFFu : 0u;
                            const uint32_t pc = (uint32_t)__popc(cb);
                            const uint32_t incl = wave_inclusive_scan(pc), excl = incl - pc;
                            const uint32_t key = mine ? (k << 16) | (uint32_t)row : 0x80000000u + (uint32_t)lane;
                            const uint32_t key_prev = (uint32_t)__builtin_amdgcn_update_dpp((int)0xFFFFFFFFu, (int)key, 0x138, 0xf, 0xf, false);
                            const bool starts = lane == 0 || key_prev != key;
                            const uint32_t seg = wave_inclusive_max(starts ? excl : 0u);
                            if (mine) {
                                uint32_t at = cw[(row - r0) * kMaxStrips + (int)k] + (excl - seg);
                                const uint32_t ge = v.x & 0xFFFFu;
                                uint32_t w = cb;
                                while (w) {
                                    const int b = __ffs((int)w) - 1;
                                    w &= w - 1;
                                    const uint32_t x = ge * kGroupPx + (uint32_t)b;
                                    uint32_t I;
                                    if constexpr (sizeof(PixelT) == 2) {
                                        const uint32_t pw = b < 2 ? px.x : b < 4 ? px.y : b < 6 ? px.z : px.w;
                                        I = (b & 1) ? pw >> 16 : pw & 0xFFFFu;
                                    } else {
                                        I = b == 0 ? px.x : b == 1 ? px.y : b == 2 ? px.z : px.w;
                                    }
                                    if (at < a.cap) gi[at] = I;
                                    if (a.need_lists && at < a.cap) gk[at] = (uint32_t)row * W + x;
                                    if (at < (uint32_t)kChainLdsEntries) s_x[at] = (uint16_t)x;
                                    if (a.dense_bytes) sbytes[(uint64_t)row * a.bpitch + x] = 1;
                                    ++at;
                                }
                            }
                            __builtin_amdgcn_wave_barrier();
                            const uint32_t key_next = (uint32_t)__builtin_amdgcn_update_dpp((int)0xFFFFFFFFu, (int)key, 0x130, 0xf, 0xf, false);
                            if (mine && (lane == 63 || key_next != key)) cw[(row - r0) * kMaxStrips + (int)k] += incl - seg;
                            __builtin_amdgcn_wave_barrier();
                        }
                    }
                }
            }
        }
        if (run_flag) n = 0;
        __syncthreads();
        FFS_STOP_AFTER(A, 5);
        FFS_PHASE_TS(A, 3);
// ... 424 lines not shown
```

### fast-feedback-service_amd/csrc/kernels_stream.hpp

```cpp
#pragma once
#include "kernels_threshold.hpp"

#ifndef FFS_IMG_LOAD_AUX
#define FFS_IMG_LOAD_AUX 0
#endif

namespace ffsamd {

constexpr int kSQWords = 32;

__device__ __forceinline__ bool exact_predicate(const ThresholdArgs& a, uint32_t m, unsigned long long sx,
                                                unsigned long long sy, uint32_t pc) {
    const double src = (double)pc;
    if (!((int)m >= a.min_count && src > a.threshold)) return false;
    if (a.max_valid >= 0 && (long long)pc > a.max_valid) return false;
    const double md = (double)m, xd = (double)sx, yd = (double)sy;
    const double t0 = md * yd;
    const double t1 = xd * xd;
    const double t2 = xd * (md - 1.0);
    const double av = (t0 - t1) - t2;
    const double bv = md * src - xd;
    const double cv = (xd * a.nsig_b) * __builtin_sqrt(2.0 * (md - 1.0));
    const double dv = a.nsig_s * __builtin_sqrt(xd * md);
    return av > cv && bv > dv;
// ... 3 lines not shown
                                                       unsigned long long sy, uint32_t pc, bool& certain) {
    const double src = (double)pc;
    const bool ok = (int)m >= a.min_count && src > a.threshold && !(a.max_valid >= 0 && (long long)pc > a.max_valid);
    const double md = (double)m, xd = (double)sx, yd = (double)sy;
    const double av = (md * yd - xd * xd) - xd * (md - 1.0);
    const double bv = md * src - xd;
    const bool pos = av > 0.0 && bv > 0.0;
    const double a2 = av * av, c2 = (a.nsig_b2 * (xd * xd)) * (2.0 * (md - 1.0));
    const double b2 = bv * bv, d2 = a.nsig_s2 * (xd * md);
    constexpr double kEps = 9.094947017729282e-13;
    const bool disp_yes = a2 > c2 + c2 * kEps, disp_no = a2 < c2 - c2 * kEps;
    const bool sig_yes = b2 > d2 + d2 * kEps, sig_no = b2 < d2 - d2 * kEps;
    certain = !(ok && pos) || ((disp_yes || disp_no) && (sig_yes || sig_no));
    return ok && pos && disp_yes && sig_yes;
}

__device__ __forceinline__ bool int_predicate(const ThresholdArgs& a, uint32_t m, uint32_t x, uint32_t y, uint32_t pc, bool& certain) {
    const bool ok = (int)m >= a.min_count && pc > a.thr_floor && !(a.max_valid >= 0 && (long long)pc > a.max_valid);
    const unsigned long long my = (unsigned long long)m * y;
    const unsigned long long xx = (unsigned long long)x * (x + m - 1u);
    const int32_t bv = (int32_t)__umul24(m, pc) - (int32_t)x;
    const bool pos = my > xx && bv > 0;
    const unsigned long long av = my - xx;
    const unsigned long long c2 = (unsigned long long)(a.ib2 * 2u * (m - 1u)) * (unsigned long long)(x * x);
    const bool small = av < (1ull << 25);
    const unsigned long long a2 = (unsigned long long)(uint32_t)av * (uint32_t)av;
    const bool disp_yes = !small || a2 > c2;
    const bool disp_close = small && (a2 > c2 ? a2 - c2 : c2 - a2) < 16ull;
    const uint32_t bu = (uint32_t)bv;
    const unsigned long long b2 = (unsigned long long)bu * bu;
    const unsigned long long d2 = (unsigned long long)a.is2 * __umul24(x, m);
    const bool sig_yes = b2 > d2;
    const bool sig_close = (b2 > d2 ? b2 - d2 : d2 - b2) < 16ull;
    certain = !(ok && pos && (disp_close || sig_close));
    return ok && pos && disp_yes && sig_yes;
}

__device__ __forceinline__ bool dispersion_only(const ThresholdArgs& a, uint32_t m, unsigned long long sx, unsigned long long sy) {
    const double md = (double)m, xd = (double)sx, yd = (double)sy;
    const double t0 = md * yd;
    const double t1 = xd * xd;
    const double t2 = xd * (md - 1.0);
    const double av = (t0 - t1) - t2;
    const double cv = (xd * a.nsig_b) * __builtin_sqrt(2.0 * (md - 1.0));
    return av > cv;
}
__device__ __forceinline__ bool dispersion_only_nosqrt(const ThresholdArgs& a, uint32_t m, unsigned long long sx, unsigned long long sy,
                                                       bool& certain) {
    certain = true;
    const double md = (double)m, xd = (double)sx, yd = (double)sy;
    const double av = (md * yd - xd * xd) - xd * (md - 1.0);
    if (!(av > 0.0)) return false;
    const double a2 = av * av, c2 = (a.nsig_b2 * (xd * xd)) * (2.0 * (md - 1.0));
    constexpr double kEps = 9.094947017729282e-13;
    const bool yes = a2 > c2 + c2 * kEps, no = a2 < c2 - c2 * kEps;
    certain = yes || no;
    return yes;
}

__device__ __forceinline__ uint32_t dpp_shr_add(uint32_t from_neighbour, uint32_t addend) {
    return (uint32_t)__builtin_amdgcn_update_dpp(0, (int)from_neighbour, 0x138, 0xf, 0xf, true) + addend;
}
__device__ __forceinline__ uint32_t dpp_shl_add(uint32_t from_neighbour, uint32_t addend) {
    return (uint32_t)__builtin_amdgcn_update_dpp(0, (int)from_neighbour, 0x130, 0xf, 0xf, true) + addend;
}


template <int KAHEAD, bool EXT = false, bool DENSE = false>
__global__ __launch_bounds__(64, 4) void k_stream_u16(const ThresholdArgs a) {
    __shared__ uint32_t s_q[kSQWords][kQCap];
    __shared__ uint16_t s_list[kQCap * 8];

    const int lane = threadIdx.x;
    if (a.dbg_prio & 1) __builtin_amdgcn_s_setprio(3);
    int strip, band;
    const bool real = stream_unit(a, blockIdx.x, strip, band);
    if constexpr (!EXT)
        if (a.handoff && blockIdx.x == gridDim.x - 1 && blockIdx.y == gridDim.y - 1 && lane == 0)
            __hip_atomic_store(a.handoff, a.handoff_seq, __ATOMIC_RELEASE, __HIP_MEMORY_SCOPE_SYSTEM);
    if (!real) return;
    [[maybe_unused]] const uint32_t slot = log_slot(a, blockIdx.y, (uint32_t)band, (uint32_t)strip);
    const int f0 = blockIdx.y * a.group_frames;
    const int nf = min(a.group_frames, a.n_frames - f0);
    const int yb0 = band_first_row(band, a.band_rows, a.band_rows2, a.band_split);
    const int yb1 = min(band_first_row(band + 1, a.band_rows, a.band_rows2, a.band_split), a.H);

    const int gsep = a.gpf + 1;
    const int G = strip * kSOwned + lane - 1;
    const int fl = G >= 0 ? G / gsep : 0;
    const int g = G - fl * gsep;
    const bool active = G >= 0 && fl < nf && g < a.gpf;
    const bool owned = active && lane >= 1 && lane <= kSOwned;
    const uint32_t my_fg = ((uint32_t)fl << 16) | (uint32_t)g;

    const rsrc_t r_img = make_rsrc((const uint8_t*)a.image + (uint64_t)f0 * a.frame_stride,
                                   (uint32_t)((uint64_t)(nf - 1) * a.frame_stride + (uint64_t)a.H * a.pitch));
    const rsrc_t r_info = make_rsrc(a.ginfo, (uint32_t)(a.H + kInfoExtraRows) * a.gpitch);
    const rsrc_t r_sb = make_rsrc(a.strong_bytes + (uint64_t)f0 * a.bytes_frame_stride,
                                  (uint32_t)((uint64_t)nf * a.bytes_frame_stride));
    const rsrc_t r_cb = make_rsrc((EXT ? a.dplane : a.bits) + (uint64_t)f0 * a.plane_frame_stride, (uint32_t)((uint64_t)nf * a.plane_frame_stride));
    constexpr uint32_t kOob = 0x80000000u;
    const uint32_t off_px = active ? (uint32_t)((uint64_t)fl * a.frame_stride) + (uint32_t)g * 16u : kOob;
    const uint32_t off_info = active ? (uint32_t)g * 4u : kOob;
    uint32_t off_byte_st;
    {
        const uint32_t lpf = a.bpitch >> 7;
        const uint32_t u = (uint32_t)strip * 4u + ((uint32_t)lane >> 4);
        const uint32_t fz = u / lpf, cz = u - fz * lpf;
        off_byte_st = fz < (uint32_t)nf ? (uint32_t)((uint64_t)fz * a.bytes_frame_stride) + cz * 128u + ((uint32_t)lane & 15u) * 8u : kOob;
    }

    const int total = (yb1 - yb0) + (FFS_DBG(a, 1024) ? 0 : 6);
    const float kS = a.kS;

    constexpr int NS = 7 + KAHEAD;
    uint32_t ring[NS][4];
    uint32_t rinfo[NS];
    uint32_t col[8], colq[8];
    uint32_t M[4] = {0, 0, 0, 0};
    uint32_t mprev = 0;
    typedef float f32x2 __attribute__((ext_vector_type(2)));
    [[maybe_unused]] f32x2 ext_c1 = {0.0f, 0.0f}, ext_c2 = {0.0f, 0.0f};
#pragma unroll
    for (int s = 0; s < NS; ++s) {
        rinfo[s] = 0;
#pragma unroll
        for (int q = 0; q < 4; ++q) ring[s][q] = 0;
    }
#pragma unroll
    for (int j = 0; j < 8; ++j) { col[j] = 0; colq[j] = 0; }
    const unsigned long long owned_mask = __builtin_amdgcn_ballot_w64(owned);

    auto fetch = [&](int slot, int i) {
        const int yin = yb0 - 3 + i;
        const uint32_t prow = (uint32_t)min(max(yin, 0), a.H - 1);
        const uint32_t irow = (uint32_t)min(max(yin, 0), a.H + kInfoExtraRows - 1);
        const u32x4 v = __builtin_amdgcn_raw_buffer_load_b128(r_img, off_px, prow * a.pitch, FFS_IMG_LOAD_AUX);
        ring[slot][0] = v[0]; ring[slot][1] = v[1]; ring[slot][2] = v[2]; ring[slot][3] = v[3];
        rinfo[slot] = __builtin_amdgcn_raw_buffer_load_b32(r_info, off_info | (yin < 0 ? kOob : 0u), (FFS_DBG(a, 64) ? 8u : irow) * a.gpitch, 0);
    };

    auto mask_row = [&](int slot, int slot_before) {
        if (__ballot(rinfo[slot] != rinfo[slot_before]) != 0ull) {
            const uint32_t mb = rinfo[slot] & 0xFFu;
            if (__ballot(mb != mprev) != 0ull) {
#pragma unroll
                for (int q = 0; q < 4; ++q)
                    M[q] = ((uint32_t)__builtin_amdgcn_sbfe((int)mb, 2 * q, 1) & 0xFFFFu)
                         | ((uint32_t)__builtin_amdgcn_sbfe((int)mb, 2 * q + 1, 1) & 0xFFFF0000u);
                mprev = mb;
            }
            if constexpr (EXT) {
                const uint32_t mmin = (rinfo[slot] >> 8) & 0xFFu, mmax = (rinfo[slot] >> 16) & 0xFFu;
                const float mm1 = (float)mmin - 1.0f;
                const float c1 = (float)mmax * 1.0000019073486328125f;
                const float c2 = (mm1 + a.kB * __builtin_amdgcn_sqrtf(2.0f * mm1)) * 0.99999952316284179688f;
                ext_c1 = f32x2{c1, c1};
                ext_c2 = f32x2{c2, c2};
            }
        }
#pragma unroll
        for (int q = 0; q < 4; ++q) {
            ring[slot][q] &= M[q];
            asm("" : "+v"(ring[slot][q]));
        }
    };

    auto push = [&](int s, int so) {
// ... 268 lines not shown
                    if (qn + nfl > kQCap) drain();
                    if constexpr (EXT) {
                        if (flag && !FFS_DBG(a, 32)) {
                            const uint32_t rank = __builtin_amdgcn_mbcnt_hi((uint32_t)(fm >> 32), __builtin_amdgcn_mbcnt_lo((uint32_t)fm, 0u));
                            const int e = qn + (int)rank;
#pragma unroll
                            for (int w = 0; w < 8; ++w) {
                                s_q[w][e] = Wn[w];
                                s_q[16 + w][e] = ys[w];
                            }
#pragma unroll
                            for (int w = 0; w < 4; ++w) s_q[8 + w][e] = ring[sc][w];
                            s_q[15][e] = info;
                            s_q[30][e] = ((uint32_t)yout << 6) | (uint32_t)lane; s_q[31][e] = my_fg;
                        }
                    } else {
                    const uint32_t QL5 = from_left(colq[5]), QL6 = from_left(colq[6]), QL7 = from_left(colq[7]);
                    const uint32_t QR0 = from_right(colq[0]), QR1 = from_right(colq[1]), QR2 = from_right(colq[2]);
                    if (flag && !FFS_DBG(a, 32)) {
                        const uint32_t rank = __builtin_amdgcn_mbcnt_hi((uint32_t)(fm >> 32), __builtin_amdgcn_mbcnt_lo((uint32_t)fm, 0u));
                        const int e = qn + (int)rank;
#pragma unroll
                        for (int w = 0; w < 8; ++w) {
                            s_q[w][e] = Wn[w];
                            s_q[19 + w][e] = colq[w];
                        }
#pragma unroll
                        for (int w = 0; w < 4; ++w) s_q[8 + w][e] = ring[sc][w];
                        s_q[15][e] = info;
                        s_q[16][e] = QL5; s_q[17][e] = QL6; s_q[18][e] = QL7;
                        s_q[27][e] = QR0; s_q[28][e] = QR1; s_q[29][e] = QR2;
                        s_q[30][e] = ((uint32_t)yout << 6) | (uint32_t)lane; s_q[31][e] = my_fg;
                    }
                    }
                    qn += nfl;
                }
            }
        }
    }
rows_done:
    if (qn > 0) drain();
    if constexpr (!EXT) if (a.wlog) {
        flush_log();
        if (lane == 0) a.wlog_n[slot] = FFS_DBG(a, 512) ? 0u : nlog;
    }
}
template <typename PixelT, bool EXT = false>
__global__ __launch_bounds__(256) void k_bright_fix(const ThresholdArgs a) {
    if (blockIdx.x == 0 && threadIdx.x == 0 && *a.bright_n > a.bright_cap) atomicOr(a.overflow, kOvfBrightList);
    const uint32_t n = min(*a.bright_n, a.bright_cap);
    for (uint32_t e = blockIdx.x * 256 + threadIdx.x; e < n; e += gridDim.x * 256) {
        const uint2 r = a.bright_list[e];
        const uint32_t frame = r.x >> 16, x = r.x & 0xFFFFu, y = r.y;
        const uint8_t* img = (const uint8_t*)a.image + (uint64_t)frame * a.frame_stride;
        if (exact_strong<PixelT, EXT>(a, img, (int)x, (int)y)) {
            uint8_t* plane = (EXT ? a.dplane : a.bits) + (uint64_t)frame * a.plane_frame_stride + (uint64_t)y * a.mpitch;
            atomicOr(reinterpret_cast<uint32_t*>(plane) + (x >> 5), 1u << (x & 31u));
            if (!EXT) {
                atomicAdd(a.tile_counts + (uint64_t)frame * a.n_tiles + y / (uint32_t)kTileRows, 1u);
                const uint32_t ob = y * a.occ_spr + (x >> 7);
                atomicOr(a.occ + (uint64_t)frame * a.occ_frame_words + (ob >> 5), 1u << (ob & 31u));
            }
        }
    }
}


constexpr int kS4Words = 32;

template <int KAHEAD, bool DENSE = false>
__global__ __launch_bounds__(64, 4) void k_stream_u32(const ThresholdArgs a) {
    __shared__ uint32_t s_q[kS4Words][kQCap];
    __shared__ uint16_t s_list[kQCap * 4];

    const int lane = threadIdx.x;
    int strip, band;
    const bool real = stream_unit(a, blockIdx.x, strip, band);
    if (a.handoff && blockIdx.x == gridDim.x - 1 && blockIdx.y == gridDim.y - 1 && lane == 0)
        __hip_atomic_store(a.handoff, a.handoff_seq, __ATOMIC_RELEASE, __HIP_MEMORY_SCOPE_SYSTEM);
    if (!real) return;
    const uint32_t slot = log_slot(a, blockIdx.y, (uint32_t)band, (uint32_t)strip);
    const int f0 = blockIdx.y * a.group_frames;
    const int nf = min(a.group_frames, a.n_frames - f0);
    const int yb0 = band_first_row(band, a.band_rows, a.band_rows2, a.band_split);
    const int yb1 = min(band_first_row(band + 1, a.band_rows, a.band_rows2, a.band_split), a.H);

    const int gsep = a.gpf + 1;
    const int G = strip * kSOwned + lane - 1;
    const int fl = G >= 0 ? G / gsep : 0;
    const int g = G - fl * gsep;
    const bool active = G >= 0 && fl < nf && g < a.gpf;
    const bool owned = active && lane >= 1 && lane <= kSOwned;

    const rsrc_t r_img = make_rsrc((const uint8_t*)a.image + (uint64_t)f0 * a.frame_stride,
                                   (uint32_t)((uint64_t)(nf - 1) * a.frame_stride + (uint64_t)a.H * a.pitch));
    const rsrc_t r_info = make_rsrc(a.ginfo, (uint32_t)(a.H + kInfoExtraRows) * a.gpitch);
    const rsrc_t r_sb = make_rsrc(a.strong_bytes + (uint64_t)f0 * a.bytes_frame_stride,
                                  (uint32_t)((uint64_t)nf * a.bytes_frame_stride));
    constexpr uint32_t kOob = 0x80000000u;
    const uint32_t off_px = active ? (uint32_t)((uint64_t)fl * a.frame_stride) + (uint32_t)g * 16u : kOob;
    const uint32_t off_info = active ? (uint32_t)g * 4u : kOob;
    uint32_t off_byte_st;
    {
        const uint32_t lpf = a.bpitch >> 7;
        const uint32_t u = (uint32_t)strip * 2u + ((uint32_t)lane >> 4);
        const uint32_t fz = u / lpf, cz = u - fz * lpf;
        off_byte_st = (lane < 32 && fz < (uint32_t)nf) ? (uint32_t)((uint64_t)fz * a.bytes_frame_stride) + cz * 128u + ((uint32_t)lane & 15u) * 8u : kOob;
    }

    const int total = (yb1 - yb0) + 6;
    const float kS = a.kS;

    constexpr int NS = 7 + KAHEAD;
    uint32_t ring[NS][4];
    uint32_t rinfo[NS];
    uint32_t col[4];
    long long colq[4];
    uint32_t M[4] = {0, 0, 0, 0};
    uint32_t mprev = 0;
    uint32_t bighist = 0;
#pragma unroll
    for (int s = 0; s < NS; ++s) {
        rinfo[s] = 0;
#pragma unroll
        for (int q = 0; q < 4; ++q) ring[s][q] = 0;
    }
#pragma unroll
    for (int j = 0; j < 4; ++j) { col[j] = 0; colq[j] = 0; }
    const unsigned long long owned_mask = __builtin_amdgcn_ballot_w64(owned);

    auto fetch = [&](int slot, int i) {
        const int yin = yb0 - 3 + i;
        const uint32_t prow = (uint32_t)min(max(yin, 0), a.H - 1);
        const uint32_t irow = (uint32_t)min(max(yin, 0), a.H + kInfoExtraRows - 1);
        const u32x4 v = __builtin_amdgcn_raw_buffer_load_b128(r_img, off_px, prow * a.pitch, FFS_IMG_LOAD_AUX);
        ring[slot][0] = v[0]; ring[slot][1] = v[1]; ring[slot][2] = v[2]; ring[slot][3] = v[3];
        rinfo[slot] = __builtin_amdgcn_raw_buffer_load_b32(r_info, off_info | (yin < 0 ? kOob : 0u), irow * a.gpitch, 0);
    };

    auto mask_row = [&](int slot, int slot_before) {
        if (__ballot(rinfo[slot] != rinfo[slot_before]) != 0ull) {
            const uint32_t mb = rinfo[slot] & 0xFu;
            if (__ballot(mb != mprev) != 0ull) {
#pragma unroll
                for (int q = 0; q < 4; ++q) M[q] = (uint32_t)__builtin_amdgcn_sbfe((int)mb, q, 1);
                mprev = mb;
            }
        }
#pragma unroll
        for (int q = 0; q < 4; ++q) ring[slot][q] &= M[q];
    };

    auto push = [&](int s, int so) {
        const uint32_t big = ((ring[s][0] | ring[s][1]) | (ring[s][2] | ring[s][3])) >> 24 ? 1u : 0u;
        bighist = (bighist & ~((1u << s) | (1u << so))) | (big << s);
#pragma unroll
        for (int q = 0; q < 4; ++q) {
            const int32_t t = (int32_t)(ring[s][q] - ring[so][q]), u = (int32_t)(ring[s][q] + ring[so][q]);
            col[q] += (uint32_t)t;
            colq[q] += (long long)t * (long long)u;
        }
    };

    int qn = 0;
    uint32_t nlog = 0;
    uint32_t nbuf = 0;
    uint32_t lbuf[6] = {0, 0, 0, 0, 0, 0};
    auto flush_log = [&]() {
// ... 227 lines not shown
```

### fast-feedback-service_amd/csrc/launch_geometry.hpp

```cpp
#pragma once
#include <stddef.h>
#include <stdint.h>

#include <algorithm>
#include <cmath>

#include "tuning.hpp"

#if defined(__HIPCC__)
#define FFS_HD __host__ __device__
#else
#define FFS_HD
#endif

namespace ffsamd {

struct Layout {
    int W, H;
    int pitch_px;
    uint32_t pitch;
    uint32_t mpitch;
    uint32_t bpitch;
    uint64_t frame_stride;
    uint64_t plane_frame_stride;
    uint64_t bytes_frame_stride;
};
inline Layout default_layout(uint32_t width, uint32_t height, int pixel_bytes) {
    Layout L{};
    L.W = (int)width;
    L.H = (int)height;
    L.pitch_px = ((int)width + 127) / 128 * 128;
    L.pitch = (uint32_t)L.pitch_px * (uint32_t)pixel_bytes;
    L.mpitch = (uint32_t)L.pitch_px / 8;
    L.bpitch = (uint32_t)L.pitch_px;
    L.frame_stride = (uint64_t)L.pitch * height;
    L.plane_frame_stride = (uint64_t)L.mpitch * height;
    L.bytes_frame_stride = (uint64_t)L.bpitch * height;
    return L;
}
inline uint32_t ginfo_pitch(const Layout& L, int pixel_bytes) { return (uint32_t)L.pitch_px * (uint32_t)pixel_bytes / 4; }
inline int groups_per_row(const Layout& L, int pixel_bytes) { return pixel_bytes == 2 ? (L.W + 7) / 8 : (L.W + 3) / 4; }

constexpr int kSOwned = 62;
constexpr int kWinOwned = 62;
constexpr int kExtOwnedPx = 56;
constexpr int kBandMaxRows = 128;
constexpr int kBandCw = 1024;
constexpr int kMergeMaxBands = 128;
constexpr int kBandSplitRows = 96;

struct StreamGeometry {
    int group_frames;
    int n_groups;
    int n_strips, n_bands;
    int band_rows, band_rows2, band_split;
};
inline StreamGeometry stream_geometry(const Layout& L, int pixel_bytes, uint64_t frame_stride, uint32_t n_frames, const Tuning& tune) {
    StreamGeometry a{};
    const int gpf = groups_per_row(L, pixel_bytes);
    {
        const uint64_t per_frame = std::max<uint64_t>(frame_stride, L.bytes_frame_stride);
        a.group_frames = (int)std::max<uint64_t>(1, std::min<uint64_t>(n_frames, ((1ull << 31) - 1) / per_frame));
        a.group_frames = std::min(a.group_frames, tune.frames_per_group);
        a.n_groups = ((int)n_frames + a.group_frames - 1) / a.group_frames;
        const long long lanes = (long long)a.group_frames * (gpf + 1);
        const long long lines = (long long)a.group_frames * (L.bpitch / 128);
        const int lines_per_wave = pixel_bytes == 2 ? 4 : 2;
        a.n_strips = (int)std::max<long long>((lanes + kSOwned - 1) / kSOwned, (lines + lines_per_wave - 1) / lines_per_wave);
        const long long per_band = std::max<long long>(1, (long long)a.n_strips * a.n_groups);
        long long nb = std::max<long long>(1, std::min<long long>(tune.target_waves / per_band, L.H / 72));
        if (nb >= 8) nb = nb / 8 * 8;
        if (tune.stream_bands > 0) nb = std::max<long long>(1, std::min<long long>(tune.stream_bands, L.H / 8));
        a.band_rows = (int)std::min<long long>(1024, (L.H + nb - 1) / nb);
        a.n_bands = (L.H + a.band_rows - 1) / a.band_rows;
        a.band_rows2 = a.band_rows;
        a.band_split = a.n_bands;
        const int taper = tune.band_taper;
        if (taper > 0 && taper < 100 && nb >= 32 && nb % 8 == 0 && a.n_bands == (int)nb) {
            const int K = (int)nb / 8;
            const int K2 = 2, K1 = K - K2;
            const double h1f = (double)L.H / (8.0 * (K1 + K2 * taper / 100.0));
            int h1 = std::min(1024, (int)std::ceil(h1f));
            int h2 = (int)std::ceil((L.H / 8.0 - (double)K1 * h1) / K2);
            while (h2 < 24) { --h1; h2 = (int)std::ceil((L.H / 8.0 - (double)K1 * h1) / K2); }
            if (h1 >= h2 && h2 >= 24 && 8 * (K1 * h1 + K2 * h2) >= L.H && 8 * K1 * h1 < L.H) {
                a.band_rows = h1;
                a.band_rows2 = h2;
                a.band_split = 8 * K1;
                a.n_bands = a.band_split + (L.H - a.band_split * h1 + h2 - 1) / h2;
            }
        }
    }
    return a;
}
inline uint32_t strips_per_frame(const Layout& L, int pixel_bytes) { return (uint32_t)groups_per_row(L, pixel_bytes) / (uint32_t)kSOwned + 2u; }
inline size_t stream_log_slots(const StreamGeometry& g) { return (size_t)g.n_groups * (size_t)g.n_bands * (size_t)g.n_strips; }
inline size_t max_stream_log_slots(const Layout& L, int pixel_bytes, uint64_t frame_stride, uint32_t max_batch, const Tuning& tune) {
    size_t slots = 0;
    for (uint32_t nf = 1; nf <= max_batch; ++nf) slots = std::max(slots, stream_log_slots(stream_geometry(L, pixel_bytes, frame_stride, nf, tune)));
    return slots;
}

struct BandSplit { int sub = 1, sub_rows = 0; };
inline BandSplit band_split(const StreamGeometry& g) {
    const int rows = std::max(g.band_rows, g.band_rows2), sub = (rows + kBandSplitRows - 1) / kBandSplitRows;
    return {sub, (rows + sub - 1) / sub};
}
inline bool band_plan_holds(const StreamGeometry& g, const Layout& L, int pixel_bytes) {
    const uint32_t strips = strips_per_frame(L, pixel_bytes);
    const BandSplit split = band_split(g);
    const int sub = split.sub, sub_rows = split.sub_rows;
    return !(sub_rows > kBandMaxRows || (uint32_t)sub_rows * std::min(strips, 16u) > (uint32_t)kBandCw || g.n_bands * sub > kMergeMaxBands || L.W > 65535);
}
inline uint32_t band_slots(const StreamGeometry& g, uint32_t n_frames) { return n_frames * (uint32_t)(g.n_bands * band_split(g).sub); }
inline uint32_t max_band_slots(const Layout& L, int pixel_bytes, uint64_t frame_stride, uint32_t max_batch, const Tuning& tune) {
    uint32_t slots = 0;
    for (uint32_t nf = 1; nf <= max_batch; ++nf) slots = std::max(slots, band_slots(stream_geometry(L, pixel_bytes, frame_stride, nf, tune), nf));
    return slots;
}

struct WindowGeometry { int w_strips, w_band_rows, w_bands; };
inline WindowGeometry window_geometry(const Layout& L, uint32_t n_frames, int ky) {
    WindowGeometry a{};
    {
        const int g8 = (L.W + 7) / 8;
        a.w_strips = (g8 + kWinOwned - 1) / kWinOwned;
        const long long per_band = std::max<long long>(1, (long long)a.w_strips * n_frames);
        const int min_rows = std::max(32, 6 * (2 * ky + 1));
        const long long nb = std::max<long long>(1, std::min<long long>(16384 / per_band, std::max(1, L.H / min_rows)));
        a.w_band_rows = (int)((L.H + nb - 1) / nb + 7) / 8 * 8;
        a.w_bands = (L.H + a.w_band_rows - 1) / a.w_band_rows;
    }
    return a;
}

struct ExtGeometry { int ext_strips, ext_band_rows, ext_bands; };
inline ExtGeometry ext_geometry(const Layout& L, uint32_t n_frames) {
    ExtGeometry a{};
    a.ext_strips = (L.pitch_px + kExtOwnedPx - 1) / kExtOwnedPx;
    {
        const long long ext_target = 8192;
        long long er = ((long long)L.H * a.ext_strips * n_frames + 4 * ext_target - 1) / (4 * ext_target);
        er = std::max<long long>(64, std::min<long long>(er, 256));
        a.ext_band_rows = (int)er;
        a.ext_bands = (L.H + a.ext_band_rows - 1) / a.ext_band_rows;
    }
    return a;
}

FFS_HD inline int band_first_row(int band, int band_rows, int band_rows2, int band_split) {
    return band < band_split ? band * band_rows : band_split * band_rows + (band - band_split) * band_rows2;
}
FFS_HD inline uint32_t stream_units_of(int n_bands, int n_strips) { return (uint32_t)n_bands * (uint32_t)n_strips; }
FFS_HD inline uint32_t stream_chunk_of(int n_bands, int n_strips) { return (stream_units_of(n_bands, n_strips) + 7u) / 8u; }
FFS_HD inline bool stream_unit_of(uint32_t bid, int n_bands, int n_strips, int& strip, int& band) {
    const uint32_t u = (bid & 7u) * stream_chunk_of(n_bands, n_strips) + (bid >> 3);
    band = (int)(u / (uint32_t)n_strips);
    strip = (int)(u - (uint32_t)band * (uint32_t)n_strips);
    return u < stream_units_of(n_bands, n_strips);
}
FFS_HD inline uint32_t log_slot_of(int n_bands, int n_strips, uint32_t y, uint32_t band, uint32_t strip) {
    return (y * (uint32_t)n_bands + band) * (uint32_t)n_strips + strip;
}

}
```

### fast-feedback-service_amd/csrc/tuning.hpp

```cpp
#pragma once

namespace ffsamd {

struct Tuning {
    int threshold_path = 0;
    int ext_first_pass = 2;
    int sparse_stage = 2;
    int sched = 3;
    int chain_first = 2;
    int bright_cap = 1 << 20;
    int frames_per_group = 1 << 30;
    long long target_waves = 16384;
    int stream_bands = 0;
    int dense_mask = 0;
    int occupancy_bitmap = 1;
    int direct_records = 1;
    int decode_in_dense_stream = 1;
    int ccl_grid = 32;
    int ext_erode = 2;
    int ext_e_sparse = 0;
    int ext_fused = 0;
    int ext_rest_aside = 0;
    int band_taper = 0;
    int rows_ahead = 3;
    int device_lists = 2;
    int strong_log = 1;
    int chain_runs = 1;
    int sparse_bands = 1;
    int dense_overlap = 0;
    int stream_prio = 1;
    int assembly_threads = 7;
    int wait_ahead = 1;
    int sparse_priority = 0;
    int window_kernel = 0;
#ifdef FFS_EXPERIMENTS
    struct Exp {
        int k1_debug = 0, chain_skip = 0, chain_stop = 0, dummy_us = 0, dummy_wg = 32, dummy_threads = 1024, dummy_lds = 0;
    } exp;
#endif
};

}
```

### fast-feedback-service_amd/python/ffs_amd/api.py

```python
from __future__ import annotations

import ctypes as C
import os
from dataclasses import dataclass, field

import numpy as np

_PKG = os.path.dirname(os.path.dirname(os.path.dirname(os.path.abspath(__file__))))


def lib_path() -> str:
    return os.environ.get("FFS_HIP_LIB") or os.path.join(_PKG, "libffs_hip.so")


class FfsError(RuntimeError):
    def __init__(self, code: int, msg: str):
        super().__init__(f"libffs_hip error {code}: {msg}")
        self.code = code


class Params(C.Structure):
    _fields_ = [("min_count", C.c_int32), ("nsig_b", C.c_double), ("nsig_s", C.c_double),
                ("threshold", C.c_double), ("max_valid", C.c_int64),
                ("min_spot_size", C.c_uint32), ("min_spot_size_3d", C.c_uint32),
                ("max_peak_centroid_separation", C.c_float),
                ("want_reflections", C.c_int32), ("want_strong_list", C.c_int32),
                ("want_strong_mask", C.c_int32), ("algorithm", C.c_int32), ("extended_flavour", C.c_int32),
                ("kernel_half_x", C.c_int32), ("kernel_half_y", C.c_int32)]


ALGO_DISPERSION, ALGO_DISPERSION_EXTENDED = 0, 1


class _Box(C.Structure):
    _fields_ = [("l", C.c_uint32), ("t", C.c_uint32), ("r", C.c_uint32), ("b", C.c_uint32),
                ("num_pixels", C.c_int32)]


class _Refl(C.Structure):
    _fields_ = [("x_min", C.c_uint32), ("x_max", C.c_uint32), ("y_min", C.c_uint32), ("y_max", C.c_uint32),
                ("z_min", C.c_int32), ("z_max", C.c_int32), ("num_pixels", C.c_int32),
                ("com_x", C.c_float), ("com_y", C.c_float), ("com_z", C.c_float),
                ("peak_x", C.c_uint32), ("peak_y", C.c_uint32), ("peak_z", C.c_int32),
                ("peak_intensity", C.c_uint32), ("peak_centroid_distance", C.c_float),
                ("flags", C.c_uint32), ("sum_intensity", C.c_uint64)]


class _FrameResult(C.Structure):
    _fields_ = [("frame_id", C.c_int64), ("num_strong_pixels", C.c_uint32),
                ("num_strong_pixels_filtered", C.c_uint32), ("n_components", C.c_uint32),
                ("n_boxes", C.c_uint32), ("boxes", C.POINTER(_Box)),
                ("n_reflections", C.c_uint32), ("reflections", C.POINTER(_Refl)),
                ("n_filtered_size", C.c_uint32), ("n_filtered_sep", C.c_uint32),
                ("strong_k", C.POINTER(C.c_uint32)), ("strong_intensity", C.POINTER(C.c_uint32)),
                ("strong_mask", C.POINTER(C.c_uint8))]


BOX_DT = np.dtype([("l", "<u4"), ("t", "<u4"), ("r", "<u4"), ("b", "<u4"), ("num_pixels", "<i4")])
REFL_DT = np.dtype([("x_min", "<u4"), ("x_max", "<u4"), ("y_min", "<u4"), ("y_max", "<u4"),
                    ("z_min", "<i4"), ("z_max", "<i4"), ("num_pixels", "<i4"),
                    ("com_x", "<f4"), ("com_y", "<f4"), ("com_z", "<f4"),
                    ("peak_x", "<u4"), ("peak_y", "<u4"), ("peak_z", "<i4"),
                    ("peak_intensity", "<u4"), ("peak_centroid_distance", "<f4"),
                    ("flags", "<u4"), ("sum_intensity", "<u8")])
assert REFL_DT.itemsize == C.sizeof(_Refl) and BOX_DT.itemsize == C.sizeof(_Box)
_FRAME_RESULT_DT = np.dtype({"names": ["frame_id", "num_strong_pixels", "num_strong_pixels_filtered", "n_components", "n_boxes", "n_reflections"],
                             "formats": ["<i8", "<u4", "<u4", "<u4", "<u4", "<u4"],
                             "offsets": [getattr(_FrameResult, f).offset for f in
                                         ("frame_id", "num_strong_pixels", "num_strong_pixels_filtered", "n_components", "n_boxes", "n_reflections")],
                             "itemsize": C.sizeof(_FrameResult)})

CODEC_BSLZ4 = 0
CODEC_BYTE_OFFSET = 1

EXPORTS = [
    "ffs_default_params", "ffs_device_count", "ffs_device_name", "ffs_device_total_mem",
    "ffs_ctx_create", "ffs_ctx_destroy", "ffs_last_error", "ffs_ctx_set_mask",
    "ffs_ctx_apply_resolution_mask", "ffs_ctx_get_mask", "ffs_ctx_set_params",
    "ffs_stream_create", "ffs_stream_destroy", "ffs_stream_host_buffer", "ffs_submit",
    "ffs_submit_device", "ffs_ctx_device_layout", "ffs_wait", "ffs_stream_batch_arrays", "ffs_stream_timings",
    "ffs_submit_compressed", "ffs_decode_only", "ffs_submit_encoded", "ffs_decode_only_encoded", "ffs_stream_spot_centres", "ffs_bench_threshold", "ffs_bench_hbm", "ffs_stream_debug_planes", "ffs_stream_debug_bitplane", "ffs_selftest_sqrt", "ffs_stack3d_create",
    "ffs_stack3d_destroy", "ffs_stack3d_add_batch", "ffs_stack3d_add_slice", "ffs_stack3d_finish", "ffs_stack3d_signals", "ffs_stack3d_last_finish_ms", "ffs_multi_init", "ffs_multi_transport",
    "ffs_ctx_set_tuning", "ffs_bench_pipeline", "ffs_device_numa_node", "ffs_stream_reserve_host", "ffs_stream_last_path", "ffs_multi_gather_rows",
]

_lib = None


def load_library():
    global _lib
    if _lib is None:
        p = lib_path()
        if not os.path.exists(p):
            raise RuntimeError(f"{p} is missing: run `make hip` or __graft_entry__.build(). "
                               "There is no CPU fallback for the product path.")
        L = C.CDLL(p)
        L.ffs_last_error.restype = C.c_char_p
        L.ffs_last_error.argtypes = [C.c_void_p]
        L.ffs_ctx_create.argtypes = [C.c_int, C.c_uint32, C.c_uint32, C.c_int, C.c_uint32, C.c_uint32,
                                     C.POINTER(C.c_void_p)]
        L.ffs_ctx_destroy.argtypes = [C.c_void_p]
        L.ffs_ctx_set_mask.argtypes = [C.c_void_p, C.c_void_p]
        L.ffs_ctx_get_mask.argtypes = [C.c_void_p, C.c_void_p]
        L.ffs_ctx_set_params.argtypes = [C.c_void_p, C.POINTER(Params)]
        L.ffs_ctx_set_tuning.argtypes = [C.c_void_p, C.c_char_p, C.c_longlong]
        L.ffs_bench_pipeline.argtypes = [C.POINTER(C.c_void_p), C.c_uint32, C.c_void_p, C.c_size_t, C.c_size_t, C.c_uint32,
                                         C.c_uint32, C.c_int64, C.POINTER(C.c_uint64), C.POINTER(C.c_uint64)]
        L.ffs_device_numa_node.argtypes = [C.c_int]
        L.ffs_stream_reserve_host.argtypes = [C.c_void_p, C.c_size_t]
        L.ffs_ctx_apply_resolution_mask.argtypes = [C.c_void_p] + [C.c_float] * 8
        L.ffs_ctx_device_layout.argtypes = [C.c_void_p, C.POINTER(C.c_size_t), C.POINTER(C.c_size_t)]
        L.ffs_stream_create.argtypes = [C.c_void_p, C.POINTER(C.c_void_p)]
        L.ffs_stream_destroy.argtypes = [C.c_void_p]
        L.ffs_stream_host_buffer.argtypes = [C.c_void_p, C.POINTER(C.c_void_p), C.POINTER(C.c_size_t)]
        L.ffs_submit.argtypes = [C.c_void_p, C.c_void_p, C.c_uint32, C.c_int64]
        L.ffs_submit_device.argtypes = [C.c_void_p, C.c_void_p, C.c_size_t, C.c_size_t, C.c_uint32, C.c_int64]
        L.ffs_wait.argtypes = [C.c_void_p, C.POINTER(C.POINTER(_FrameResult)), C.POINTER(C.c_uint32)]
        L.ffs_stream_timings.argtypes = [C.c_void_p, C.POINTER(C.c_float)]
        L.ffs_stream_last_path.argtypes = [C.c_void_p, C.POINTER(C.c_uint32), C.POINTER(C.c_uint32)]
        L.ffs_stream_batch_arrays.argtypes = [C.c_void_p, C.POINTER(C.c_void_p), C.POINTER(C.c_uint32),
                                              C.POINTER(C.c_void_p), C.POINTER(C.c_uint32)]
        L.ffs_bench_threshold.argtypes = [C.c_void_p, C.c_void_p, C.c_size_t, C.c_size_t, C.c_uint32,
                                          C.c_uint32, C.POINTER(C.c_float), C.POINTER(C.c_float)]
        L.ffs_multi_init.argtypes = [C.POINTER(C.c_int), C.c_int, C.c_char_p]
        L.ffs_multi_transport.restype = C.c_char_p
        L.ffs_bench_hbm.argtypes = [C.c_void_p, C.c_uint32, C.POINTER(C.c_float), C.POINTER(C.c_float)]
        L.ffs_stream_debug_planes.argtypes = [C.c_void_p, C.POINTER(C.c_void_p), C.POINTER(C.c_size_t),
                                              C.POINTER(C.c_size_t)]
        L.ffs_stream_spot_centres.argtypes = [C.c_void_p, C.c_void_p, C.c_uint32, C.POINTER(C.c_uint32)]
        L.ffs_submit_compressed.argtypes = [C.c_void_p, C.c_void_p, C.c_void_p, C.c_uint32, C.c_int64]
        L.ffs_decode_only.argtypes = [C.c_void_p, C.c_void_p, C.c_void_p, C.c_uint32, C.c_uint32,
                                      C.POINTER(C.c_float), C.c_void_p]
        L.ffs_submit_encoded.argtypes = [C.c_void_p, C.c_int, C.c_void_p, C.c_void_p, C.c_uint32, C.c_int64]
        L.ffs_decode_only_encoded.argtypes = [C.c_void_p, C.c_int, C.c_void_p, C.c_void_p, C.c_uint32, C.c_uint32,
                                              C.POINTER(C.c_float), C.c_void_p]
        L.ffs_stack3d_signals.argtypes = [C.c_void_p] * 7
        L.ffs_stream_debug_bitplane.argtypes = [C.c_void_p, C.c_uint32, C.c_int, C.c_void_p]
        L.ffs_selftest_sqrt.argtypes = [C.c_void_p, C.c_uint64, C.c_uint64, C.POINTER(C.c_uint64)]
        L.ffs_device_name.argtypes = [C.c_int, C.c_char_p, C.c_size_t]
        L.ffs_device_total_mem.argtypes = [C.c_int, C.POINTER(C.c_uint64)]
        L.ffs_stack3d_create.argtypes = [C.c_void_p, C.c_uint64, C.POINTER(C.c_void_p)]
        L.ffs_stack3d_destroy.argtypes = [C.c_void_p]
        L.ffs_stack3d_add_batch.argtypes = [C.c_void_p, C.c_void_p]
        L.ffs_stack3d_add_slice.argtypes = [C.c_void_p, C.c_int64, C.c_void_p, C.c_void_p, C.c_uint32]
        L.ffs_stack3d_finish.argtypes = [C.c_void_p, C.POINTER(C.POINTER(_Refl)), C.POINTER(C.c_uint32),
                                         C.POINTER(C.c_uint32), C.POINTER(C.c_uint32), C.POINTER(C.c_uint32)]
        _lib = L
    return _lib


def device_count() -> int:
    return load_library().ffs_device_count()


def device_name(device: int = 0) -> str:
    buf = C.create_string_buffer(256)
    rc = load_library().ffs_device_name(device, buf, 256)
    if rc != 0:
        raise FfsError(rc, "no such device")
    return buf.value.decode()


def default_params() -> Params:
    p = Params()
    load_library().ffs_default_params(C.byref(p))
    return p


@dataclass
class FrameResult:
    frame_id: int
    num_strong_pixels: int
    num_strong_pixels_filtered: int
    n_components: int
    boxes: np.ndarray
    reflections: np.ndarray | None
    n_filtered_size: int
    n_filtered_sep: int
    strong_k: np.ndarray | None = None
    strong_intensity: np.ndarray | None = None
    strong_mask: np.ndarray | None = None
    extra: dict = field(default_factory=dict)

    @property
    def n_spots_total(self) -> int:
        return len(self.boxes)


def _copy_array(ptr, n, ctype_struct, dt):
    if n == 0 or not ptr:
        return np.zeros(0, dt)
    raw = C.string_at(C.cast(ptr, C.c_void_p), n * C.sizeof(ctype_struct))
    return np.frombuffer(raw, dtype=dt).copy()


class Context:
    def __init__(self, width: int, height: int, dtype=np.uint16, max_batch: int = 1,
                 device: int = 0, max_strong_per_frame: int = 0):
        self._lib = load_library()
        self.W, self.H = int(width), int(height)
        self.dtype = np.dtype(dtype)
        assert self.dtype in (np.dtype(np.uint16), np.dtype(np.uint32))
        self.max_batch = int(max_batch)
        self.device = device
        h = C.c_void_p()
        rc = self._lib.ffs_ctx_create(device, self.W, self.H, self.dtype.itemsize, self.max_batch,
                                      max_strong_per_frame, C.byref(h))
        if rc != 0:
            raise FfsError(rc, self._lib.ffs_last_error(None).decode())
        self._h = h
        self.params = default_params()

    def _check(self, rc):
        if rc != 0:
            raise FfsError(rc, self._lib.ffs_last_error(self._h).decode())

    def set_mask(self, mask: np.ndarray | None):
        if mask is None:
            self._check(self._lib.ffs_ctx_set_mask(self._h, None))
            return
        m = np.ascontiguousarray(mask, dtype=np.uint8)
        assert m.shape == (self.H, self.W)
        self._check(self._lib.ffs_ctx_set_mask(self._h, m.ctypes.data_as(C.c_void_p)))

    def get_mask(self) -> np.ndarray:
        m = np.empty((self.H, self.W), np.uint8)
        self._check(self._lib.ffs_ctx_get_mask(self._h, m.ctypes.data_as(C.c_void_p)))
        return m

    def apply_resolution_mask(self, wavelength, distance_m, beam_center_x_px, beam_center_y_px,
                              pixel_size_x_m, pixel_size_y_m, dmin=-1.0, dmax=-1.0):
        self._check(self._lib.ffs_ctx_apply_resolution_mask(
            self._h, wavelength, distance_m, beam_center_x_px, beam_center_y_px,
            pixel_size_x_m, pixel_size_y_m, dmin, dmax))

    def set_params(self, **kw):
        for k, v in kw.items():
            if not hasattr(self.params, k):
                raise AttributeError(k)
            setattr(self.params, k, v)
        self._check(self._lib.ffs_ctx_set_params(self._h, C.byref(self.params)))

    def set_tuning(self, **kw):
        for k, v in kw.items():
            self._check(self._lib.ffs_ctx_set_tuning(self._h, k.encode(), int(v)))

    def selftest_sqrt(self, begin: int, end: int) -> int:
        out = C.c_uint64()
        self._check(self._lib.ffs_selftest_sqrt(self._h, begin, end, C.byref(out)))
        return out.value

    def device_layout(self):
        pitch, stride = C.c_size_t(), C.c_size_t()
        self._check(self._lib.ffs_ctx_device_layout(self._h, C.byref(pitch), C.byref(stride)))
        return pitch.value, stride.value

    def stream(self) -> "Stream":
        return Stream(self)

    def close(self):
        if self._h:
            self._lib.ffs_ctx_destroy(self._h)
            self._h = None

    def __del__(self):
        try:
            self.close()
        except Exception:
            pass


class Stream:
    def __init__(self, ctx: Context):
        self.ctx = ctx
        self._lib = ctx._lib
        h = C.c_void_p()
        ctx._check(self._lib.ffs_stream_create(ctx._h, C.byref(h)))
        self._h = h
        self._batch_wants = (False, False)

    def host_buffer(self) -> np.ndarray:
        p, n = C.c_void_p(), C.c_size_t()
        self.ctx._check(self._lib.ffs_stream_host_buffer(self._h, C.byref(p), C.byref(n)))
        frames = self.ctx.max_batch * self.ctx.H * self.ctx.W * self.ctx.dtype.itemsize
        assert n.value >= frames, "the staging area was reserved smaller than max_batch frames (reserve_host)"
        buf = (C.c_uint8 * frames).from_address(p.value)
        return np.frombuffer(buf, dtype=self.ctx.dtype).reshape(self.ctx.max_batch, self.ctx.H, self.ctx.W)

    def reserve_host(self, nbytes: int):
        self.ctx._check(self._lib.ffs_stream_reserve_host(self._h, nbytes))

    def host_bytes(self) -> np.ndarray:
        p, n = C.c_void_p(), C.c_size_t()
        self.ctx._check(self._lib.ffs_stream_host_buffer(self._h, C.byref(p), C.byref(n)))
        return np.frombuffer((C.c_uint8 * n.value).from_address(p.value), dtype=np.uint8)

    def _chunk_args(self, chunks):
        keep = [np.frombuffer(c, np.uint8) if not isinstance(c, np.ndarray) else c for c in chunks]
        ptrs = (C.c_void_p * len(keep))(*[k.ctypes.data for k in keep])
        sizes = (C.c_size_t * len(keep))(*[k.size for k in keep])
        return keep, ptrs, sizes

    def submit_compressed(self, chunks, first_frame_id: int = 0):
        self._keep, ptrs, sizes = self._chunk_args(chunks)
        self.ctx._check(self._lib.ffs_submit_compressed(self._h, ptrs, sizes, len(self._keep), first_frame_id))
        self._snapshot()

    def process_compressed(self, chunks, first_frame_id: int = 0):
        self.submit_compressed(chunks, first_frame_id)
        return self.wait()

    def submit_encoded(self, chunks, codec: int, first_frame_id: int = 0):
        self._keep, ptrs, sizes = self._chunk_args(chunks)
        self.ctx._check(self._lib.ffs_submit_encoded(self._h, codec, ptrs, sizes, len(self._keep), first_frame_id))
        self._snapshot()

    def process_encoded(self, chunks, codec: int, first_frame_id: int = 0):
        self.submit_encoded(chunks, codec, first_frame_id)
        return self.wait()

    def decode_only(self, chunks, iters: int = 1, want_frames: bool = True, codec: int = CODEC_BSLZ4):
        keep, ptrs, sizes = self._chunk_args(chunks)
        ms = C.c_float()
        out = np.empty((len(keep), self.ctx.H, self.ctx.W), self.ctx.dtype) if want_frames else None
        self.ctx._check(self._lib.ffs_decode_only_encoded(self._h, codec, ptrs, sizes, len(keep), iters, C.byref(ms),
                                                          out.ctypes.data_as(C.c_void_p) if want_frames else None))
        return ms.value, out

# ... 210 lines not shown
```

### include/ffs_hip.h

```cpp
#ifndef FFS_HIP_H
#define FFS_HIP_H

#include <stddef.h>
#include <stdint.h>

#ifdef __cplusplus
extern "C" {
#endif

#pragma GCC visibility push(default)

#define FFS_OK 0
#define FFS_ERR_INVALID (-1)
#define FFS_ERR_DEVICE (-2)
#define FFS_ERR_NOMEM (-3)
#define FFS_ERR_OVERFLOW (-4)
#define FFS_ERR_NODEVICE (-5)

typedef struct ffs_ctx ffs_ctx;
typedef struct ffs_stream ffs_stream;
typedef struct ffs_stack3d ffs_stack3d;

typedef struct {
    int32_t min_count;
// ... 34 lines not shown
    uint32_t peak_x, peak_y;
    int32_t peak_z;
    uint32_t peak_intensity;
    float peak_centroid_distance;
    uint32_t flags;
    uint64_t sum_intensity;
} ffs_reflection;

typedef struct {
    int64_t frame_id;
    uint32_t num_strong_pixels;
    uint32_t num_strong_pixels_filtered;
    uint32_t n_components;
    uint32_t n_boxes;
    const ffs_box *boxes;
    uint32_t n_reflections;
    const ffs_reflection *reflections;
    uint32_t n_filtered_size, n_filtered_sep;
    const uint32_t *strong_k;
    const uint32_t *strong_intensity;
    const uint8_t *strong_mask;
} ffs_frame_result;

int ffs_device_count(void);
int ffs_device_name(int device, char *buf, size_t buflen);
int ffs_device_total_mem(int device, uint64_t *bytes);

int ffs_ctx_create(int device, uint32_t width, uint32_t height, int pixel_bytes,
                   uint32_t max_batch, uint32_t max_strong_per_frame, ffs_ctx **out);
void ffs_ctx_destroy(ffs_ctx *ctx);
const char *ffs_last_error(const ffs_ctx *ctx);

int ffs_ctx_set_mask(ffs_ctx *ctx, const uint8_t *host_mask);

int ffs_ctx_apply_resolution_mask(ffs_ctx *ctx, float wavelength, float distance_m,
                                  float beam_center_x_px, float beam_center_y_px,
                                  float pixel_size_x_m, float pixel_size_y_m, float dmin,
                                  float dmax);
int ffs_ctx_get_mask(ffs_ctx *ctx, uint8_t *host_mask);

int ffs_ctx_set_params(ffs_ctx *ctx, const ffs_params *p);

int ffs_ctx_set_tuning(ffs_ctx *ctx, const char *key, long long value);

int ffs_stream_create(ffs_ctx *ctx, ffs_stream **out);
void ffs_stream_destroy(ffs_stream *s);

int ffs_stream_host_buffer(ffs_stream *s, void **ptr, size_t *bytes);
int ffs_stream_reserve_host(ffs_stream *s, size_t bytes);

int ffs_submit(ffs_stream *s, const void *host_pixels, uint32_t n_frames,
               int64_t first_frame_id);
int ffs_submit_device(ffs_stream *s, const void *device_pixels, size_t pitch_bytes,
                      size_t frame_stride_bytes, uint32_t n_frames, int64_t first_frame_id);
int ffs_ctx_device_layout(const ffs_ctx *ctx, size_t *pitch_bytes, size_t *frame_stride_bytes);

int ffs_submit_compressed(ffs_stream *s, const void *const *chunks, const size_t *chunk_bytes,
                          uint32_t n_frames, int64_t first_frame_id);
int ffs_decode_only(ffs_stream *s, const void *const *chunks, const size_t *chunk_bytes,
                    uint32_t n_frames, uint32_t iters, float *ms_decode, void *host_out);

#define FFS_CODEC_BSLZ4 0
#define FFS_CODEC_BYTE_OFFSET 1
int ffs_submit_encoded(ffs_stream *s, int codec, const void *const *chunks, const size_t *chunk_bytes,
                       uint32_t n_frames, int64_t first_frame_id);
int ffs_decode_only_encoded(ffs_stream *s, int codec, const void *const *chunks, const size_t *chunk_bytes,
                            uint32_t n_frames, uint32_t iters, float *ms_decode, void *host_out);

int ffs_wait(ffs_stream *s, const ffs_frame_result **results, uint32_t *n_results);

int ffs_stream_batch_arrays(ffs_stream *s, const ffs_box **boxes, uint32_t *n_boxes,
                            const ffs_reflection **reflections, uint32_t *n_reflections);

int ffs_stream_timings(ffs_stream *s, float ms[5]);

#define FFS_PATH_WAVE_LOGS 1u
#define FFS_PATH_FRAME_CHAIN 2u
#define FFS_PATH_BANDS 4u
#define FFS_PATH_RUNS 8u
#define FFS_PATH_GRID_KERNELS 16u
#define FFS_PATH_EXTENDED 32u
#define FFS_PATH_WINDOW 64u
int ffs_stream_last_path(ffs_stream *s, uint32_t *path_bits, uint32_t *reruns);

int ffs_stream_spot_centres(ffs_stream *s, float *rows4, uint32_t cap, uint32_t *n_written);

int ffs_bench_threshold(ffs_stream *s, const void *device_pixels, size_t pitch_bytes,
                        size_t frame_stride_bytes, uint32_t n_frames, uint32_t iters,
                        float *ms_dense, float *ms_rest);
int ffs_bench_pipeline(ffs_stream *const *streams, uint32_t n_streams, const void *device_pixels,
                       size_t pitch_bytes, size_t frame_stride_bytes, uint32_t n_frames, uint32_t steps,
                       int64_t first_frame_id, uint64_t *n_boxes, uint64_t *n_strong_pixels);
int ffs_bench_hbm(ffs_stream *s, uint32_t iters, float *read_gbps, float *mix_gbps);
int ffs_stream_debug_planes(ffs_stream *s, const uint8_t **device_strong_bytes,
                            size_t *mask_pitch, size_t *mask_frame_stride);
int ffs_stream_debug_bitplane(ffs_stream *s, uint32_t frame_in_batch, int which, uint8_t *host_out);

int ffs_selftest_sqrt(ffs_ctx *ctx, uint64_t begin, uint64_t end, uint64_t *sum_of_bits);

int ffs_stack3d_create(ffs_ctx *ctx, uint64_t max_total_strong, ffs_stack3d **out);
void ffs_stack3d_destroy(ffs_stack3d *st);
int ffs_stack3d_add_batch(ffs_stack3d *st, ffs_stream *s);
int ffs_stack3d_add_slice(ffs_stack3d *st, int64_t frame_id, const uint32_t *k,
                          const uint32_t *intensity, uint32_t n);
int ffs_stack3d_finish(ffs_stack3d *st, const ffs_reflection **reflections,
                       uint32_t *n_reflections, uint32_t *n_calculated,
                       uint32_t *n_filtered_size, uint32_t *n_filtered_sep);
int ffs_multi_init(const int *devices, int n_devices, const char *transport);
const char *ffs_multi_transport(void);
int ffs_multi_gather_rows(ffs_stream *const *streams, uint32_t n_streams, uint32_t root, float *rows4_out, uint32_t cap,
                          uint32_t *n_rows);
int ffs_device_numa_node(int device);
int ffs_stack3d_last_finish_ms(const ffs_stack3d *st, float *ms);
int ffs_stack3d_signals(ffs_stack3d *st, const uint32_t **x, const uint32_t **y, const int32_t **z,
                        const uint32_t **intensity, const int32_t **reflection, uint64_t *n);

#pragma GCC visibility pop

#ifdef __cplusplus
}
#endif
#endif
```

Before: 113,900 frames/s.

## Plan band rows from detector mask runs via a device band table

Replaces the arithmetic band-row formula in the kernels with a per-band row table uploaded to device memory. An optional planner, controlled by a new mask_bands tuning flag that defaults to off, cuts bands at long fully masked row gaps so that no work is spent on masked rows, and seam merging skips band pairs that do not touch. It also makes band and strip wave-uniform with readfirstlane. With default settings the uniform table is used, which adds one global load per block and some host-side table management.

```diff
diff --git a/fast-feedback-service_amd/csrc/ffs_bench.hip b/fast-feedback-service_amd/csrc/ffs_bench.hip
--- a/fast-feedback-service_amd/csrc/ffs_bench.hip
+++ b/fast-feedback-service_amd/csrc/ffs_bench.hip
@@ -18,8 +18,10 @@
         if (rc != FFS_OK) return rc;
     }
     s->ext_e_clean = false;
-    const StreamGeometry geo = batch_stream_geometry(s, fstride, n_frames);
-    ThresholdArgs ta = make_threshold_args(s, device_pixels, pitch, fstride, n_frames, geo, Rerun{});
+    const BandRows* band_tab = nullptr;
+    const StreamGeometry geo = batch_stream_geometry(s, fstride, n_frames, Rerun{}, &band_tab);
+    if (!band_tab) return FFS_ERR_NOMEM;
+    ThresholdArgs ta = make_threshold_args(s, device_pixels, pitch, fstride, n_frames, geo, band_tab, Rerun{});
     if (!ext && !win_default(c->params) && !window_kernel_for(s, ta)) {
         c->err = "ffs_bench_threshold: threshold_path 2 with a window other than 3,3 has no dense kernel to time";
         return FFS_ERR_INVALID;
diff --git a/fast-feedback-service_amd/csrc/ffs_context.hip b/fast-feedback-service_amd/csrc/ffs_context.hip
--- a/fast-feedback-service_amd/csrc/ffs_context.hip
+++ b/fast-feedback-service_amd/csrc/ffs_context.hip
@@ -292,6 +292,7 @@
         pool->owner.unlock();
         delete pool;
     }
+    drop_band_tables(c);
     if (c->d_maskbits) (void)hipFree(c->d_maskbits);
     if (c->d_ginfo) (void)hipFree(c->d_ginfo);
     if (c->d_mmap) (void)hipFree(c->d_mmap);
@@ -319,6 +320,18 @@
                            L.pitch_px, c->d_mmap, c->d_ginfo, gpitch);
     HIP_TRY(c, hipGetLastError());
     HIP_TRY(c, hipDeviceSynchronize());
+    std::vector<uint8_t> bits(L.plane_frame_stride);
+    HIP_TRY(c, hipMemcpy(bits.data(), c->d_maskbits, bits.size(), hipMemcpyDeviceToHost));
+    std::vector<RowRun> runs;
+    for (int y = 0; y < L.H; ++y) {
+        const uint8_t* row = bits.data() + (size_t)y * L.mpitch;
+        bool any = false;
+        for (uint32_t i = 0; i < L.mpitch && !any; ++i) any = row[i] != 0;
+        if (!any) continue;
+        if (!runs.empty() && runs.back().end == y) runs.back().end = y + 1;
+        else runs.push_back({y, y + 1});
+    }
+    set_mask_rows(c, std::move(runs));
     return FFS_OK;
 }
 
@@ -455,6 +468,7 @@
     else if (k == "ext_e_sparse") { if ((ok = in(0, 1))) t.ext_e_sparse = (int)value; }
     else if (k == "ext_rest_aside") { if ((ok = in(0, 1))) t.ext_rest_aside = (int)value; }
     else if (k == "band_taper") { if ((ok = in(0, 99))) t.band_taper = (int)value; }
+    else if (k == "mask_bands") { if ((ok = in(0, 1))) t.mask_bands = (int)value; }
     else if (k == "rows_ahead") { if ((ok = in(2, 4))) t.rows_ahead = (int)value; }
     else if (k == "ccl_grid") { if ((ok = in(1, 1024))) t.ccl_grid = (int)value; }
     else {
diff --git a/fast-feedback-service_amd/csrc/ffs_device.h b/fast-feedback-service_amd/csrc/ffs_device.h
--- a/fast-feedback-service_amd/csrc/ffs_device.h
+++ b/fast-feedback-service_amd/csrc/ffs_device.h
@@ -34,7 +34,7 @@
     uint32_t mpitch, bpitch;
     uint64_t plane_frame_stride, bytes_frame_stride;
     int n_strips, band_rows, n_bands, n_tiles;
-    int band_rows2, band_split;
+    const BandRows* band_tab;
     float kS;
     float kB;
     int min_count;
@@ -57,7 +57,6 @@
     int gpf;
     int n_frames;
     int group_frames;
-    int s_strips, s_band_rows, s_bands;
     uint32_t* bright_n;
     uint2* bright_list;
     uint32_t bright_cap;
@@ -81,7 +80,14 @@
 __host__ __device__ inline uint32_t stream_units(const ThresholdArgs& a) { return stream_units_of(a.n_bands, a.n_strips); }
 __host__ __device__ inline uint32_t stream_chunk(const ThresholdArgs& a) { return stream_chunk_of(a.n_bands, a.n_strips); }
 __device__ __forceinline__ bool stream_unit(const ThresholdArgs& a, uint32_t bid, int& strip, int& band) {
-    return stream_unit_of(bid, a.n_bands, a.n_strips, strip, band);
+    const bool real = stream_unit_of(bid, a.n_bands, a.n_strips, strip, band);
+    band = __builtin_amdgcn_readfirstlane(band);
+    strip = __builtin_amdgcn_readfirstlane(strip);
+    return real;
+}
+__device__ __forceinline__ BandRows band_rows_of(const ThresholdArgs& a, int band) {
+    const BandRows r = a.band_tab[__builtin_amdgcn_readfirstlane(band)];
+    return {r.first, min(r.end, a.H)};
 }
 __host__ __device__ inline uint32_t log_slot(const ThresholdArgs& a, uint32_t y, uint32_t band, uint32_t strip) {
     return log_slot_of(a.n_bands, a.n_strips, y, band, strip);
diff --git a/fast-feedback-service_amd/csrc/ffs_internal.hpp b/fast-feedback-service_amd/csrc/ffs_internal.hpp
--- a/fast-feedback-service_amd/csrc/ffs_internal.hpp
+++ b/fast-feedback-service_amd/csrc/ffs_internal.hpp
@@ -109,6 +109,16 @@
     std::atomic<uint32_t> chain_ev_next{0};
     std::atomic<int> chain_ev_newest{-1};
     bool chain_ok = false;
+    struct BandTable {
+        int u_bands, u_rows, u_rows2, u_split;
+        bool masked;
+        StreamGeometry plan;
+        std::vector<BandRows> rows;
+        BandRows* d_rows;
+    };
+    std::vector<RowRun> mask_runs;
+    std::vector<BandTable> band_tables;
+    std::mutex band_mu;
     std::atomic<AssemblyPool*> assembly{nullptr};
     std::atomic<AheadThread*> ahead{nullptr};
     ThreadError err;
@@ -306,8 +316,11 @@
 int ensure_host_staging(ffs_stream* s, size_t bytes);
 size_t default_staging_bytes(const ffs_stream* s);
 bool chain_prepare_device();
-StreamGeometry batch_stream_geometry(const ffs_stream* s, size_t fstride, uint32_t n_frames);
-ThresholdArgs make_threshold_args(ffs_stream* s, const void* img, size_t pitch, size_t fstride, uint32_t n_frames, const StreamGeometry& g, const Rerun& how);
+StreamGeometry batch_stream_geometry(const ffs_stream* s, size_t fstride, uint32_t n_frames, const Rerun& how, const BandRows** d_rows, std::vector<BandRows>* host_rows = nullptr);
+void drop_band_tables(ffs_ctx* c);
+void set_mask_rows(ffs_ctx* c, std::vector<RowRun>&& runs);
+ThresholdArgs make_threshold_args(ffs_stream* s, const void* img, size_t pitch, size_t fstride, uint32_t n_frames, const StreamGeometry& g, const BandRows* band_tab,
+                                  const Rerun& how);
 int check_layout(ffs_stream* s, size_t pitch, size_t fstride, uint32_t n_frames);
 int ensure_extended_buffers(ffs_stream* s);
 int enqueue_batch(ffs_stream* s, const void* d_img, size_t pitch, size_t fstride, uint32_t n, const ffs_params* snapshot = nullptr,
diff --git a/fast-feedback-service_amd/csrc/ffs_submit.hip b/fast-feedback-service_amd/csrc/ffs_submit.hip
--- a/fast-feedback-service_amd/csrc/ffs_submit.hip
+++ b/fast-feedback-service_amd/csrc/ffs_submit.hip
@@ -19,6 +19,15 @@
     return e1 == hipSuccess && e2 == hipSuccess && e3 == hipSuccess && e4 == hipSuccess && e5 == hipSuccess;
 }
 
+static int batch_threshold_path(const ffs_ctx* c, const Rerun& how) { return how.threshold_path >= 0 ? how.threshold_path : c->tune.threshold_path; }
+static bool batch_dense_mask(const ffs_ctx* c, const ffs_params& p, const Rerun& how) {
+    bool dense = p.want_strong_mask || c->tune.dense_mask || batch_threshold_path(c, how) != 0;
+#ifdef FFS_EXPERIMENTS
+    if (c->tune.exp.k1_debug & 16) dense = true;
+    if (c->tune.exp.k1_debug & 8) dense = false;
+#endif
+    return dense;
+}
 static void set_buffers(ThresholdArgs& a, const ffs_stream* s, const void* img, size_t pitch, size_t fstride, const Rerun& how) {
     const ffs_ctx* c = s->ctx;
     const Layout& L = c->L;
@@ -38,7 +47,7 @@
     a.plane_frame_stride = L.plane_frame_stride;
     a.bytes_frame_stride = L.bytes_frame_stride;
     a.n_tiles = c->n_tiles;
-    a.bright_to_plane = how.threshold_path >= 0 ? how.threshold_path : c->tune.threshold_path;
+    a.bright_to_plane = batch_threshold_path(c, how);
     a.overflow = s->d_overflow;
     a.bright_n = s->d_tile_counts + tile_counts_bytes(s) / 4 - 1;
     a.bright_list = s->d_bright;
@@ -46,11 +55,9 @@
     a.occ = s->d_occ;
     a.occ_frame_words = occ_frame_words(L);
     a.occ_spr = L.mpitch / 16;
-    a.dense_mask = (p.want_strong_mask || c->tune.dense_mask || a.bright_to_plane) ? 1 : 0;
+    a.dense_mask = batch_dense_mask(c, p, how) ? 1 : 0;
 #ifdef FFS_EXPERIMENTS
     a.dbg = c->tune.exp.k1_debug;
-    if (a.dbg & 16) a.dense_mask = 1;
-    if (a.dbg & 8) a.dense_mask = 0;
 #endif
     a.dbg_prio = c->tune.stream_prio;
     a.ginfo = c->d_ginfo;
@@ -86,14 +93,13 @@
     a.w_kB = (std::isfinite(p.nsig_b) && p.nsig_b <= 1024.0) ? (float)(p.nsig_b * p.nsig_b * (1.0 - 1.0 / 65536.0)) : 0.0f;
     a.ext_flavour = p.extended_flavour;
 }
-static void set_geometry(ThresholdArgs& a, uint32_t n_frames, const StreamGeometry& g, const WindowGeometry& w, const ExtGeometry& e) {
+static void set_geometry(ThresholdArgs& a, uint32_t n_frames, const StreamGeometry& g, const BandRows* band_tab, const WindowGeometry& w, const ExtGeometry& e) {
     a.n_frames = (int)n_frames;
     a.group_frames = g.group_frames;
     a.n_strips = g.n_strips;
     a.n_bands = g.n_bands;
-    a.band_rows = g.band_rows;
-    a.band_rows2 = g.band_rows2;
-    a.band_split = g.band_split;
+    a.band_rows = std::max(g.band_rows, g.band_rows2);
+    a.band_tab = band_tab;
     a.w_strips = w.w_strips;
     a.w_band_rows = w.w_band_rows;
     a.w_bands = w.w_bands;
@@ -101,14 +107,84 @@
     a.ext_band_rows = e.ext_band_rows;
     a.ext_bands = e.ext_bands;
 }
-StreamGeometry batch_stream_geometry(const ffs_stream* s, size_t fstride, uint32_t n_frames) {
-    return stream_geometry(s->ctx->L, s->ctx->pixel_bytes, fstride, n_frames, s->ctx->tune);
-}
-ThresholdArgs make_threshold_args(ffs_stream* s, const void* img, size_t pitch, size_t fstride, uint32_t n_frames, const StreamGeometry& g, const Rerun& how) {
+static const ffs_ctx::BandTable* band_table_for(ffs_ctx* c, const StreamGeometry& u, bool masked) {
+    const ffs_ctx::BandTable* t = nullptr;
+    for (const auto& e : c->band_tables)
+        if (e.u_bands == u.n_bands && e.u_rows == u.band_rows && e.u_rows2 == u.band_rows2 && e.u_split == u.band_split && e.masked == masked) t = &e;
+    if (!t) {
+        ffs_ctx::BandTable e{u.n_bands, u.band_rows, u.band_rows2, u.band_split, masked, u, {}, nullptr};
+        if (masked) e.plan = band_plan(u, c->L, c->pixel_bytes, c->mask_runs.data(), c->mask_runs.size(), e.rows);
+        else uniform_band_table(u, c->L.H, e.rows);
+        if (hipMalloc(reinterpret_cast<void**>(&e.d_rows), e.rows.size() * sizeof(BandRows)) != hipSuccess
+            || hipMemcpy(e.d_rows, e.rows.data(), e.rows.size() * sizeof(BandRows), hipMemcpyHostToDevice) != hipSuccess) {
+            (void)hipGetLastError();
+            if (e.d_rows) (void)hipFree(e.d_rows);
+            c->err = "hipMalloc(band table) failed";
+            return nullptr;
+        }
+        c->band_tables.push_back(std::move(e));
+        t = &c->band_tables.back();
+    }
+    return t;
+}
+static void drop_band_tables_locked(ffs_ctx* c) {
+    for (auto& t : c->band_tables)
+        if (t.d_rows) (void)hipFree(t.d_rows);
+    c->band_tables.clear();
+}
+void drop_band_tables(ffs_ctx* c) {
+    std::lock_guard<std::mutex> lock(c->band_mu);
+    drop_band_tables_locked(c);
+}
+void set_mask_rows(ffs_ctx* c, std::vector<RowRun>&& runs) {
+    std::lock_guard<std::mutex> lock(c->band_mu);
+    drop_band_tables_locked(c);
+    c->mask_runs = std::move(runs);
+    for (uint32_t nf = 1; nf <= c->max_batch; ++nf) {
+        const StreamGeometry u = stream_geometry(c->L, c->pixel_bytes, c->L.frame_stride, nf, c->tune);
+        (void)band_table_for(c, u, false);
+        if (c->tune.mask_bands != 0 && c->tune.band_taper == 0) (void)band_table_for(c, u, true);
+    }
+}
+static StreamGeometry planned_stream_geometry(ffs_ctx* c, const ffs_params& p, size_t fstride, uint32_t n_frames, const Rerun& how, const BandRows** d_rows,
+                                              std::vector<BandRows>* host_rows) {
+    const StreamGeometry u = stream_geometry(c->L, c->pixel_bytes, fstride, n_frames, c->tune);
+    const bool masked = c->tune.mask_bands != 0 && c->tune.band_taper == 0 && !batch_dense_mask(c, p, how);
+    std::lock_guard<std::mutex> lock(c->band_mu);
+    const ffs_ctx::BandTable* t = band_table_for(c, u, masked);
+    *d_rows = t ? t->d_rows : nullptr;
+    if (!t) return u;
+    StreamGeometry g = u;
+    g.n_bands = t->plan.n_bands;
+    g.band_rows = t->plan.band_rows;
+    g.band_rows2 = t->plan.band_rows2;
+    g.band_split = t->plan.band_split;
+    if (host_rows) *host_rows = t->rows;
+    return g;
+}
+StreamGeometry batch_stream_geometry(const ffs_stream* s, size_t fstride, uint32_t n_frames, const Rerun& how, const BandRows** d_rows, std::vector<BandRows>* host_rows) {
+    return planned_stream_geometry(s->ctx, s->batch_params, fstride, n_frames, how, d_rows, host_rows);
+}
+extern "C" int ffs_ctx_band_plan(ffs_ctx* c, uint32_t n_frames, int32_t* rows, uint32_t cap, uint32_t* n_bands) {
+    if (!c || n_frames == 0 || n_frames > c->max_batch || (!rows && cap != 0)) return FFS_ERR_INVALID;
+    HIP_TRY(c, hipSetDevice(c->device));
+    std::vector<BandRows> table;
+    const BandRows* d_rows = nullptr;
+    (void)planned_stream_geometry(c, c->params, c->L.frame_stride, n_frames, Rerun{}, &d_rows, &table);
+    if (!d_rows) return FFS_ERR_NOMEM;
+    for (size_t b = 0; b < table.size() && b < cap; ++b) {
+        rows[2 * b] = table[b].first;
+        rows[2 * b + 1] = table[b].end;
+    }
+    if (n_bands) *n_bands = (uint32_t)table.size();
+    return FFS_OK;
+}
+ThresholdArgs make_threshold_args(ffs_stream* s, const void* img, size_t pitch, size_t fstride, uint32_t n_frames, const StreamGeometry& g, const BandRows* band_tab,
+                                  const Rerun& how) {
     ThresholdArgs a{};
     set_buffers(a, s, img, pitch, fstride, how);
     set_predicate(a, s->batch_params);
-    set_geometry(a, n_frames, g, window_geometry(s->ctx->L, n_frames, a.ky), ext_geometry(s->ctx->L, n_frames));
+    set_geometry(a, n_frames, g, band_tab, window_geometry(s->ctx->L, n_frames, a.ky), ext_geometry(s->ctx->L, n_frames));
     return a;
 }
 
@@ -329,6 +405,7 @@
 
 struct BatchPlan {
     uint32_t n = 0;
+    bool ok = false;
     bool wait_upload = false;
     bool counts_were_clean = false;
     bool ext = false;
@@ -362,8 +439,10 @@
     P.counts_were_clean = !s->counts_dirty;
     P.ext = p.algorithm == FFS_ALGO_DISPERSION_EXTENDED;
     P.ext_sparse_erode = ext_sparse_erode(c->tune);
-    P.geo = batch_stream_geometry(s, fstride, n);
-    P.ta = make_threshold_args(s, d_img, pitch, fstride, n, P.geo, how);
+    const BandRows* band_tab = nullptr;
+    P.geo = batch_stream_geometry(s, fstride, n, how, &band_tab);
+    P.ok = band_tab != nullptr;
+    P.ta = make_threshold_args(s, d_img, pitch, fstride, n, P.geo, band_tab, how);
     P.window = !P.ext && window_kernel_for(s, P.ta);
     P.list_path = !P.ext && !P.ta.bright_to_plane && !P.window;
     P.want_dense_bytes = P.window ? (p.want_strong_mask || c->tune.dense_mask)
@@ -728,6 +807,7 @@
     bool ext_plane_clean = false;
     FFS_TRY(take_extended_planes(s, ext_plane_clean));
     const BatchPlan plan = plan_batch(s, d_img, pitch, fstride, n, how);
+    if (!plan.ok) return FFS_ERR_NOMEM;
     if (plan.use_log && s->band_backoff > 0 && !how.no_bands) --s->band_backoff;
     bool dense_resets = false;
     FFS_TRY(reset_for_batch(s, plan, dense_resets));
diff --git a/fast-feedback-service_amd/csrc/kernels_band.hpp b/fast-feedback-service_amd/csrc/kernels_band.hpp
--- a/fast-feedback-service_amd/csrc/kernels_band.hpp
+++ b/fast-feedback-service_amd/csrc/kernels_band.hpp
@@ -51,8 +51,9 @@
     const uint32_t l_s0 = G0 / (uint32_t)kSOwned;
     const uint32_t l_ns = min(G1 / (uint32_t)kSOwned - l_s0 + 1u, 16u);
     const uint32_t wave0 = log_slot(T, l_y, (uint32_t)band, l_s0);
-    const int sb1 = min(band_first_row(band + 1, T.band_rows, T.band_rows2, T.band_split), a.H);
-    const int yb0 = min(band_first_row(band, T.band_rows, T.band_rows2, T.band_split) + sub * B.sub_rows, sb1);
+    const BandRows band_r = band_rows_of(T, band);
+    const int sb1 = band_r.end;
+    const int yb0 = min(band_r.first + sub * B.sub_rows, sb1);
     const int yb1 = min(yb0 + B.sub_rows, sb1);
     const uint32_t rows = (uint32_t)(yb1 - yb0);
     const uint8_t* img = (const uint8_t*)a.image + (uint64_t)frame * a.frame_stride;
@@ -403,7 +404,9 @@
             uint4 ht = hdr[t];
             while ((ht.w >> 16) == 0u && t + 1 < nbands) ht = hdr[++t];
             const uint32_t nbot = h.z >> 16, ntop = (ht.w >> 16) != 0u ? ht.z & 0xFFFFu : 0u;
-            if (nbot && ntop) {
+            const uint32_t sb = b / (uint32_t)B.sub, st = t / (uint32_t)B.sub;
+            const bool touch = sb == st || T.band_tab[st].first == T.band_tab[sb].end;
+            if (nbot && ntop && touch) {
                 const uint32_t* bot = seam + ((size_t)b * 2 + 1) * kBandSeamCap;
                 const uint32_t* top = seam + ((size_t)t * 2) * kBandSeamCap;
                 const uint32_t* lbot = s_seam + (b * 2u + 1u) * kMergeSeamLds;
diff --git a/fast-feedback-service_amd/csrc/kernels_chain.hpp b/fast-feedback-service_amd/csrc/kernels_chain.hpp
--- a/fast-feedback-service_amd/csrc/kernels_chain.hpp
+++ b/fast-feedback-service_amd/csrc/kernels_chain.hpp
@@ -561,8 +561,8 @@
             uint8_t* sbytes = a.strong_bytes + (uint64_t)frame * a.bytes_frame_stride;
             const uint32_t ns = min(l_ns, (uint32_t)kMaxStrips);
             for (int band = wave; band < T.n_bands; band += kChainWaves) {
-                const int yb0 = band_first_row(band, T.band_rows, T.band_rows2, T.band_split);
-                const int yb1 = min(band_first_row(band + 1, T.band_rows, T.band_rows2, T.band_split), (int)a.H);
+                const BandRows band_r = band_rows_of(T, band);
+                const int yb0 = band_r.first, yb1 = band_r.end;
                 for (int r0 = yb0; r0 < yb1; r0 += cw_rows) {
                     const int r1 = min(r0 + cw_rows, yb1);
                     for (int i = lane; i < (r1 - r0) * kMaxStrips; i += 64) cw[i] = 0;
diff --git a/fast-feedback-service_amd/csrc/kernels_stream.hpp b/fast-feedback-service_amd/csrc/kernels_stream.hpp
--- a/fast-feedback-service_amd/csrc/kernels_stream.hpp
+++ b/fast-feedback-service_amd/csrc/kernels_stream.hpp
@@ -109,8 +109,8 @@
     [[maybe_unused]] const uint32_t slot = log_slot(a, blockIdx.y, (uint32_t)band, (uint32_t)strip);
     const int f0 = blockIdx.y * a.group_frames;
     const int nf = min(a.group_frames, a.n_frames - f0);
-    const int yb0 = band_first_row(band, a.band_rows, a.band_rows2, a.band_split);
-    const int yb1 = min(band_first_row(band + 1, a.band_rows, a.band_rows2, a.band_split), a.H);
+    const BandRows band_r = band_rows_of(a, band);
+    const int yb0 = band_r.first, yb1 = band_r.end;
 
     const int gsep = a.gpf + 1;
     const int G = strip * kSOwned + lane - 1;
@@ -545,8 +545,8 @@
     const uint32_t slot = log_slot(a, blockIdx.y, (uint32_t)band, (uint32_t)strip);
     const int f0 = blockIdx.y * a.group_frames;
     const int nf = min(a.group_frames, a.n_frames - f0);
-    const int yb0 = band_first_row(band, a.band_rows, a.band_rows2, a.band_split);
-    const int yb1 = min(band_first_row(band + 1, a.band_rows, a.band_rows2, a.band_split), a.H);
+    const BandRows band_r = band_rows_of(a, band);
+    const int yb0 = band_r.first, yb1 = band_r.end;
 
     const int gsep = a.gpf + 1;
     const int G = strip * kSOwned + lane - 1;
diff --git a/fast-feedback-service_amd/csrc/launch_geometry.hpp b/fast-feedback-service_amd/csrc/launch_geometry.hpp
--- a/fast-feedback-service_amd/csrc/launch_geometry.hpp
+++ b/fast-feedback-service_amd/csrc/launch_geometry.hpp
@@ -4,6 +4,7 @@
 
 #include <algorithm>
 #include <cmath>
+#include <vector>
 
 #include "tuning.hpp"
 
@@ -151,6 +152,91 @@
 FFS_HD inline int band_first_row(int band, int band_rows, int band_rows2, int band_split) {
     return band < band_split ? band * band_rows : band_split * band_rows + (band - band_split) * band_rows2;
 }
+struct BandRows { int first, end; };
+struct RowRun { int first, end; };
+constexpr int kBandCutRows = 7;
+
+inline void uniform_band_table(const StreamGeometry& g, int H, std::vector<BandRows>& table) {
+    table.resize((size_t)g.n_bands);
+    for (int b = 0; b < g.n_bands; ++b)
+        table[(size_t)b] = {band_first_row(b, g.band_rows, g.band_rows2, g.band_split), std::min(band_first_row(b + 1, g.band_rows, g.band_rows2, g.band_split), H)};
+}
+inline StreamGeometry band_plan(const StreamGeometry& u, const Layout& L, int pixel_bytes, const RowRun* runs, size_t n_runs, std::vector<BandRows>& table) {
+    const int H = L.H;
+    StreamGeometry g = u;
+    uniform_band_table(u, H, table);
+    if (n_runs == 0 || u.band_split != u.n_bands || u.band_rows <= 0) return g;
+    std::vector<RowRun> seg;
+    bool cut = runs[0].first >= kBandCutRows;
+    seg.push_back({cut ? runs[0].first : 0, runs[0].end});
+    for (size_t r = 1; r < n_runs; ++r) {
+        if (runs[r].first - seg.back().end >= kBandCutRows) { seg.push_back(runs[r]); cut = true; }
+        else seg.back().end = runs[r].end;
+    }
+    if (H - seg.back().end >= kBandCutRows) cut = true;
+    else seg.back().end = H;
+    if (!cut) return g;
+    auto need = [&](const RowRun& s) { return (s.end - s.first + u.band_rows - 1) / u.band_rows; };
+    for (;;) {
+        long long want = 0;
+        for (const RowRun& s : seg) want += need(s);
+        if (want <= u.n_bands || seg.size() < 2) break;
+        size_t at = 1;
+        for (size_t i = 2; i < seg.size(); ++i)
+            if (seg[i].first - seg[i - 1].end < seg[at].first - seg[at - 1].end) at = i;
+        seg[at - 1].end = seg[at].end;
+        seg.erase(seg.begin() + (long)at);
+    }
+    if (seg.size() == 1 && seg[0].first == 0 && seg[0].end == H) return g;
+    long long rows = 0;
+    for (const RowRun& s : seg) rows += s.end - s.first;
+    const size_t ns = seg.size();
+    std::vector<int> k(ns);
+    std::vector<long long> rem(ns);
+    long long left = u.n_bands;
+    for (size_t i = 0; i < ns; ++i) {
+        const long long n = seg[i].end - seg[i].first, q = (long long)u.n_bands * n;
+        k[i] = (int)std::min<long long>(n, std::max<long long>(need(seg[i]), q / rows));
+        rem[i] = q % rows;
+        left -= k[i];
+    }
+    std::vector<size_t> order(ns);
+    for (size_t i = 0; i < ns; ++i) order[i] = i;
+    std::stable_sort(order.begin(), order.end(), [&](size_t a, size_t b) { return rem[a] > rem[b]; });
+    for (bool moved = true; left > 0 && moved;) {
+        moved = false;
+        for (size_t j = 0; j < ns && left > 0; ++j)
+            if (k[order[j]] < seg[order[j]].end - seg[order[j]].first) { ++k[order[j]]; --left; moved = true; }
+    }
+    while (left < 0)
+        for (size_t j = ns; j-- > 0 && left < 0;)
+            if (k[order[j]] > need(seg[order[j]])) { --k[order[j]]; ++left; }
+    table.clear();
+    int tallest = 0;
+    for (size_t i = 0; i < ns; ++i) {
+        const int n = seg[i].end - seg[i].first, h = n / k[i], extra = n % k[i];
+        int y = seg[i].first;
+        for (int b = 0; b < k[i]; ++b) {
+            const int rows_b = h + (b < extra ? 1 : 0);
+            table.push_back({y, y + rows_b});
+            y += rows_b;
+            tallest = std::max(tallest, rows_b);
+        }
+    }
+    g.n_bands = (int)table.size();
+    g.band_rows = g.band_rows2 = tallest;
+    g.band_split = g.n_bands;
+    if (band_plan_holds(u, L, pixel_bytes) && !band_plan_holds(g, L, pixel_bytes)) {
+        uniform_band_table(u, H, table);
+        return u;
+    }
+    return g;
+}
+inline long long band_table_row_iterations(const std::vector<BandRows>& table) {
+    long long it = 0;
+    for (const BandRows& b : table) it += b.end - b.first + 6;
+    return it;
+}
 FFS_HD inline uint32_t stream_units_of(int n_bands, int n_strips) { return (uint32_t)n_bands * (uint32_t)n_strips; }
 FFS_HD inline uint32_t stream_chunk_of(int n_bands, int n_strips) { return (stream_units_of(n_bands, n_strips) + 7u) / 8u; }
 FFS_HD inline bool stream_unit_of(uint32_t bid, int n_bands, int n_strips, int& strip, int& band) {
diff --git a/fast-feedback-service_amd/csrc/tuning.hpp b/fast-feedback-service_amd/csrc/tuning.hpp
--- a/fast-feedback-service_amd/csrc/tuning.hpp
+++ b/fast-feedback-service_amd/csrc/tuning.hpp
@@ -22,6 +22,7 @@
     int ext_fused = 0;
     int ext_rest_aside = 0;
     int band_taper = 0;
+    int mask_bands = 0;
     int rows_ahead = 3;
     int device_lists = 2;
     int strong_log = 1;
diff --git a/fast-feedback-service_amd/python/ffs_amd/api.py b/fast-feedback-service_amd/python/ffs_amd/api.py
--- a/fast-feedback-service_amd/python/ffs_amd/api.py
+++ b/fast-feedback-service_amd/python/ffs_amd/api.py
@@ -82,6 +82,7 @@
     "ffs_submit_compressed", "ffs_decode_only", "ffs_submit_encoded", "ffs_decode_only_encoded", "ffs_stream_spot_centres", "ffs_bench_threshold", "ffs_bench_hbm", "ffs_stream_debug_planes", "ffs_stream_debug_bitplane", "ffs_selftest_sqrt", "ffs_stack3d_create",
     "ffs_stack3d_destroy", "ffs_stack3d_add_batch", "ffs_stack3d_add_slice", "ffs_stack3d_finish", "ffs_stack3d_signals", "ffs_stack3d_last_finish_ms", "ffs_multi_init", "ffs_multi_transport",
     "ffs_ctx_set_tuning", "ffs_bench_pipeline", "ffs_device_numa_node", "ffs_stream_reserve_host", "ffs_stream_last_path", "ffs_multi_gather_rows",
+    "ffs_ctx_band_plan",
 ]
 
 _lib = None
@@ -118,6 +119,8 @@
         L.ffs_wait.argtypes = [C.c_void_p, C.POINTER(C.POINTER(_FrameResult)), C.POINTER(C.c_uint32)]
         L.ffs_stream_timings.argtypes = [C.c_void_p, C.POINTER(C.c_float)]
         L.ffs_stream_last_path.argtypes = [C.c_void_p, C.POINTER(C.c_uint32), C.POINTER(C.c_uint32)]
+        if hasattr(L, "ffs_ctx_band_plan"):
+            L.ffs_ctx_band_plan.argtypes = [C.c_void_p, C.c_uint32, C.c_void_p, C.c_uint32, C.POINTER(C.c_uint32)]
         L.ffs_stream_batch_arrays.argtypes = [C.c_void_p, C.POINTER(C.c_void_p), C.POINTER(C.c_uint32),
                                               C.POINTER(C.c_void_p), C.POINTER(C.c_uint32)]
         L.ffs_bench_threshold.argtypes = [C.c_void_p, C.c_void_p, C.c_size_t, C.c_size_t, C.c_uint32,
@@ -244,6 +247,13 @@
     def set_tuning(self, **kw):
         for k, v in kw.items():
             self._check(self._lib.ffs_ctx_set_tuning(self._h, k.encode(), int(v)))
+
+    def band_plan(self, n_frames: int) -> np.ndarray:
+        n = C.c_uint32()
+        self._check(self._lib.ffs_ctx_band_plan(self._h, n_frames, None, 0, C.byref(n)))
+        rows = np.zeros((n.value, 2), np.int32)
+        self._check(self._lib.ffs_ctx_band_plan(self._h, n_frames, rows.ctypes.data_as(C.c_void_p), n.value, C.byref(n)))
+        return rows
 
     def selftest_sqrt(self, begin: int, end: int) -> int:
         out = C.c_uint64()
diff --git a/include/ffs_hip.h b/include/ffs_hip.h
--- a/include/ffs_hip.h
+++ b/include/ffs_hip.h
@@ -140,6 +140,7 @@
 #define FFS_PATH_EXTENDED 32u
 #define FFS_PATH_WINDOW 64u
 int ffs_stream_last_path(ffs_stream *s, uint32_t *path_bits, uint32_t *reruns);
+int ffs_ctx_band_plan(ffs_ctx *ctx, uint32_t n_frames, int32_t *rows, uint32_t cap, uint32_t *n_bands);
 
 int ffs_stream_spot_centres(ffs_stream *s, float *rows4, uint32_t cap, uint32_t *n_written);
 
```

Result: no change. 113,400 frames/s (-0.5%).
